# doubleailes/crust-render

Hardware: AMD Instinct MI355X
Metric: Mray/s (closest-hit + shadow queries) of the path-tracing integrator (higher is better)
Workload: dtype f32; 1 GPU; samples/cornellbox.usda 1920x1080, 512 spp per step per GPU-share (x1 GPUs), depth 32, triangle r=1, variance 0; 14 steps = 7168 spp; rays_total=33550217735, closest_hit=33550217735, camera_rays=14863564800, target_spp=1024

## Files before the change

crust-render_amd/__init__.py:

```python
import ctypes as C
import os
import subprocess

import numpy as np

_HERE = os.path.dirname(os.path.abspath(__file__))
LIB_PATH = os.environ.get("CRT_AMD_LIB") or os.path.join(_HERE, "libcrt_amd.so")
CSRC = os.path.join(_HERE, "csrc")

MASK_CAMERA, MASK_SHADOW, MASK_INDIRECT, MASK_ALL = 1, 2, 4, 0xFFFFFFFF
INVALID_ID = 0xFFFFFFFF
INF = float("inf")

CRT_OK = 0
_ERRORS = {-1: "CRT_ERR_BAD_ARG", -2: "CRT_ERR_BAD_ID", -3: "CRT_ERR_NO_DEVICE", -4: "CRT_ERR_STACK",
           -5: "CRT_ERR_UNSUPPORTED", -6: "CRT_ERR_NO_MEMORY"}


class CrtError(RuntimeError):
    def __init__(self, code, what=""):
        detail = ""
        try:
            detail = _lib.crt_last_error().decode() if _lib is not None else ""
        except Exception:
# ... 677 lines not shown
            lib().crt_environment_free(h)

    def __del__(self):
        try:
            self.free()
        except Exception:
            pass

    def tables(self):
        t = CrtEnvironmentTables()
        _check(lib().crt_environment_tables(self.h, C.byref(t)), "crt_environment_tables")
        w, h = int(t.width), int(t.height)
        arr = lambda p, *shape: np.ctypeslib.as_array(p, shape=shape).copy()
        return dict(width=w, height=h, id=int(t.id), marginal_integral=np.float32(t.marginal_integral),
                    marginal_func=arr(t.marginal_func, h), marginal_cdf=arr(t.marginal_cdf, h + 1),
                    conditional_func=arr(t.conditional_func, h, w), conditional_cdf=arr(t.conditional_cdf, h, w + 1),
                    conditional_integral=arr(t.conditional_integral, h),
                    light_to_world=np.array(t.light_to_world, dtype=np.float32).reshape(3, 3).T.copy(),
                    world_to_light=np.array(t.world_to_light, dtype=np.float32).reshape(3, 3).T.copy(),
                    image=np.ctypeslib.as_array(C.cast(t.image, C.POINTER(C.c_uint8)), shape=(int(t.image_bytes),)).copy())


def environment_of(d):
    env = d.get("environment")
    if env is None or isinstance(env, Environment):
        return env
    return Environment(env["width"], env["height"], env["rgb"], env.get("light_to_world"))


def make_lights(light_dicts):
    arr = (CrtLight * max(len(light_dicts), 1))()
    keep = []
    for k, d in enumerate(light_dicts):
        l = arr[k]
        if d["kind"] == "dome" and d.get("environment") is not None:
            env = environment_of(d)
            tint = np.asarray(d["radiance"], dtype=np.float32)
            _check(lib().crt_light_dome_mapped(C.byref(l), _fp(tint), env.h), "crt_light_dome_mapped")
            keep.append(env)
            continue
        l.kind = {"sphere": LIGHT_SPHERE, "rect": LIGHT_RECT, "distant": LIGHT_DISTANT,
                  "dome": LIGHT_DOME}[d["kind"]]
        l.geom_id = int(d["geom_id"])
        l.radiance[:] = [float(x) for x in d["radiance"]]
        if d["kind"] == "distant":
            l.normal[:] = [float(x) for x in d["direction"]]
            l.radius = float(d["cos_half_angle"])
            l.center[0] = float(d["solid_angle"])
        elif d["kind"] == "dome":
            pass
        elif d["kind"] == "sphere":
            l.center[:] = [float(x) for x in d["center"]]
            l.radius = float(d["radius"])
        else:
            for f in ("origin", "edge_u", "edge_v", "normal"):
                getattr(l, f)[:] = [float(x) for x in d[f]]
    arr._environments = keep
    return arr


class Renderer:

    def __init__(self, scene, materials, lights, camera, settings, rank=0, world=1):
        self.scene = scene
        n = len(materials)
        self._mats = (CrtMaterial * max(n, 1))(*materials)
        self._lights = lights if not isinstance(lights, (list, tuple)) else make_lights(lights)
        self.n_lights = len(lights)
        self.settings = settings
        cs = settings.c()
        self.h = lib().crt_renderer_new(scene.h, self._mats, n, self._lights, self.n_lights, C.byref(camera),
                                        C.byref(cs), rank, world)
        if not self.h:
            raise CrtError(-1, "crt_renderer_new")
        self.n_pix = lib().crt_renderer_pixel_count(self.h)
        self.volumes = None

    def __del__(self):
        try:
            if self.h:
                lib().crt_renderer_free(self.h)
        except Exception:
            pass

    def pixel_indices(self):
        out = np.zeros(self.n_pix, dtype=np.uint32)
        _check(lib().crt_renderer_pixel_indices(self.h, _up(out)), "crt_renderer_pixel_indices")
        return out

    def render_samples(self, sample_begin, sample_count, stream=None):
        _check(lib().crt_render_samples(self.h, sample_begin, sample_count, _stream_ptr(stream)), "crt_render_samples")

    def set_volumes(self, vol):
        _check(lib().crt_renderer_set_volumes(self.h, vol.h if vol is not None else None), "crt_renderer_set_volumes")
        self.volumes = vol

    def render_samples_stats(self, sample_begin, sample_count, stream=None):
        st = (CrtTravStats * 2)()
        _check(lib().crt_render_samples_stats(self.h, sample_begin, sample_count, _stream_ptr(stream), st),
               "crt_render_samples_stats")
        return st[0], st[1]

    def film_to(self, d_rgb, stream=None):
        _check(lib().crt_film_resolve(self.h, d_rgb.data_ptr(), _stream_ptr(stream)), "crt_film_resolve")

    def film(self):
        out = np.zeros((self.n_pix, 3), dtype=np.float32)
        _check(lib().crt_film_read(self.h, _fp(out)), "crt_film_read")
        return out

    def image(self):
        img = np.zeros((self.settings.height * self.settings.width, 3), dtype=np.float32)
        img[self.pixel_indices()] = self.film()
        return img.reshape(self.settings.height, self.settings.width, 3)

    def clear(self, stream=None):
        _check(lib().crt_film_clear(self.h, _stream_ptr(stream)), "crt_film_clear")

    def stats(self):
        s = CrtRayStats()
        _check(lib().crt_render_stats(self.h, C.byref(s)), "crt_render_stats")
        return s

    def active_pixels(self):
        return int(lib().crt_renderer_active_pixels(self.h))

    def sample_counts(self):
        out = np.zeros(self.n_pix, dtype=np.uint32)
        _check(lib().crt_renderer_sample_counts(self.h, out.ctypes.data_as(C.POINTER(C.c_uint32))), "crt_renderer_sample_counts")
        return out

    def render_adaptive(self, spp, first=None, batch=4, stream=None):
        first = first or -(-max(self.settings.min_spp, 2) // 4) * 4
        s = 0
        while s < spp and self.active_pixels() > 0:
            n = min(first if s == 0 else batch, spp - s)
            self.render_samples(s, n, stream)
            s += n
        return s

    SHADE_CLASSES = ("emissive / escaped", "base", "coat / fuzz / thin film", "transmissive / subsurface")

    def shade_class_stats(self, enable=None):
        w, l = (C.c_uint64 * 4)(), (C.c_uint64 * 4)()
        _check(lib().crt_renderer_shade_class_stats(self.h, -1 if enable is None else int(bool(enable)), w, l),
               "crt_renderer_shade_class_stats")
        return {n: (int(w[k]), (l[k] / (64.0 * w[k])) if w[k] else 0.0) for k, n in enumerate(self.SHADE_CLASSES)}

    def pipeline(self):
        out = (C.c_uint32 * 3)()
        _check(lib().crt_renderer_pipeline(self.h, out), "crt_renderer_pipeline")
        return dict(fused=bool(out[0]), wide=bool(out[1] & 1), shade_pipe=bool(out[1] & 2), root_cull=bool(out[1] & 4),
                    slim_state=bool(out[1] & 8), volumes=bool(out[1] & 16), camera_trace=bool(out[1] & 32),
                    camera_vertex=bool(out[1] & 64), grid=int(out[2]))

    def lanes(self):
        return int(lib().crt_renderer_lanes(self.h)) if hasattr(lib(), "crt_renderer_lanes") else 1

    def set_lanes(self, lanes):
        return _check(lib().crt_renderer_set_lanes(self.h, int(lanes)), "crt_renderer_set_lanes")

    def profile(self, enable=True):
        _check(lib().crt_renderer_profile(self.h, 1 if enable else 0), "crt_renderer_profile")

    def profile_read(self):
        ms = (C.c_double * 4)()
        n = (C.c_uint64 * 4)()
        _check(lib().crt_renderer_profile_read(self.h, ms, n), "crt_renderer_profile_read")
        names = ("extend", "shade", "shadow", "other")
        return {names[k]: dict(ms=float(ms[k]), launches=int(n[k])) for k in range(4)}


def scene_path(name):
    import os
    if str(name).startswith("synthetic:") or os.path.exists(name):
        return name
    base = os.path.join(os.path.dirname(os.path.dirname(os.path.abspath(__file__))), "scenes", name)
    for ext in (".usda", ".usd", ".usda.xz"):
        if os.path.exists(base + ext):
            return base + ext
    raise FileNotFoundError("no scene %r under scenes/" % name)


def load_usda(path, width=None, height=None, max_depth=None, rank=0, world=1, variance=0.0, min_spp=None, dist=None,
              timings=None, cubic_curves=False, environment_maps=False):
    from . import usda, shard
    import sys
    import time
    t0 = time.perf_counter()
    if str(path).startswith("synthetic:"):
        from . import synthetic
        parts = str(path).split(":")
        kw = dict(side=int(parts[2])) if len(parts) > 2 else {}
        desc = getattr(synthetic, parts[1])(width or 640, height or 360, **kw)
    else:
        desc = shard.import_once(path, width, height, dist, cubic_curves=cubic_curves, environment_maps=environment_maps)
    me = sys.modules[__name__]
    t1 = time.perf_counter()
    scene, materials, protos = usda.build_world(desc, me, default_material)
    t2 = time.perf_counter()
    if timings is not None:
        timings.update(import_s=t1 - t0, commit_s=t2 - t1)
    s = desc.settings
    settings = RenderSettings(s["width"], s["height"], s["max_depth"] if max_depth is None else max_depth, s["frame"],
                              s["strategy"], s["filter"], s["filter_radius"], float(variance),
                              s["min_spp"] if min_spp is None else min_spp)
    cam = make_camera(**desc.camera)
    r = Renderer(scene, materials, desc.lights, cam, settings, rank, world)
    r._protos = protos
    return r, desc

def render_with_report(path, spp=None, out_exr=None, width=None, height=None, max_depth=None, variance=None,
                       batch=16, volumes=False):
    import sys
    from . import stats as _stats
    st = _stats.RenderStats()
    me = sys.modules[__name__]
    with st.phase("Parse USD stage"):
        desc = usda.load(path, width, height, volumes=bool(volumes))
    s = desc.settings
    with st.phase("Commit acceleration structure"):
        scene, materials, protos = usda.build_world(desc, me, default_material)
        scene.memory_footprint()
    var = s["variance"] if variance is None else variance
    settings = RenderSettings(s["width"], s["height"], s["max_depth"] if max_depth is None else max_depth, s["frame"],
                              s["strategy"], s["filter"], s["filter_radius"], float(var), s["min_spp"])
    r = Renderer(scene, materials, desc.lights, make_camera(**desc.camera), settings)
    r._protos = protos
    vol = usda.build_volumes(desc, me) if volumes else None
    if vol is not None:
        r.set_volumes(vol)
    n = int(spp if spp is not None else s["spp"])
    with st.phase("Render"):
        if var > 0:
            r.render_adaptive(n, batch=batch)
        else:
            for b in range(0, n, 32):
                r.render_samples(b, min(32, n - b))
        img = r.image()
    if out_exr:
        with st.phase("Write image"):
            exr.write_exr(out_exr, img[::-1])
    _stats.for_render(scene, r, n, st)
    return img, st


load_scene = load_usda

from . import usda
from . import usdc
from . import shard
from . import exr
from . import stats
from . import shading
from . import volumes
from . import guiding
from . import synthetic
```

crust-render_amd/csrc/crt_internal.h:

```cpp
#pragma once

#include <atomic>
#include <cmath>
#include <cstddef>
#include <cstdint>
#include <memory>
#include <mutex>
#include <vector>

#include "../../include/crt.h"
#include "../../include/crt_render_volumes.h"
#include "../../include/crt_scene_image.h"

namespace crt {

struct F3 {
  float x, y, z;
  float operator[](int i) const { return i == 0 ? x : (i == 1 ? y : z); }
  float &at(int i) { return i == 0 ? x : (i == 1 ? y : z); }
};
inline F3 f3(float x, float y, float z) { return F3{x, y, z}; }
inline F3 operator+(F3 a, F3 b) { return {a.x + b.x, a.y + b.y, a.z + b.z}; }
inline F3 operator-(F3 a, F3 b) { return {a.x - b.x, a.y - b.y, a.z - b.z}; }
inline F3 operator*(F3 a, float s) { return {a.x * s, a.y * s, a.z * s}; }
// ... 182 lines not shown
inline bool wide_split(const DevScene &s, bool renderer = false) {
  if (s.direct_leaves != 0 || s.n_packets == 0) return false;
  if (s.pool_stack >= 10u) return renderer && s.n_nodes > 2048u;
  return s.n_nodes <= 1024u;
}

#ifndef CRT_POOL_STACK
#define CRT_POOL_STACK 6
#endif
#ifndef CRT_POOL_STACK_DEEP
#define CRT_POOL_STACK_DEEP 10
#endif
#ifndef CRT_POOL_STACK_WIDE
#define CRT_POOL_STACK_WIDE 3
#endif

struct EngineSelect {
  bool wide = false;
  bool wide_direct = false;
  bool direct = false;
  uint32_t lds_stack = CRT_POOL_STACK;
  uint32_t window = CRT_POOL_NODES;
  int ext_cold = (int)kColdAll;
  int path_cold = (int)kColdAll;
  bool curve = false;
  bool cubic = false;
  int curve_cold() const { return (int)((curve ? kColdCurve : 0u) | (cubic ? kColdCubic : 0u)); }
};
inline int select_engine(const DevScene &s, int want_wide, EngineSelect &e, bool renderer = false) {
  const bool has_direct_words = s.direct_leaves != 0;
  const bool curve = (s.cold & kColdCurve) != 0;
  if (curve && want_wide > 0) return CRT_ERR_UNSUPPORTED;
  if (want_wide == 1 && has_direct_words) return CRT_ERR_UNSUPPORTED;
  if (want_wide == 2 && !(has_direct_words && renderer && CRT_DIRECT_LEAVES != 0 && CRT_WIDE_DIRECT_BUILD != 0)) return CRT_ERR_UNSUPPORTED;
  const bool auto_wide_direct = !curve && want_wide < 0 && renderer && has_direct_words && CRT_DIRECT_LEAVES != 0 && CRT_WIDE_DIRECT_BUILD != 0;
  e.wide = auto_wide_direct || (want_wide < 0 ? (!curve && wide_split(s, renderer)) : want_wide != 0);
  e.wide_direct = auto_wide_direct || want_wide == 2;
  e.direct = (!e.wide || e.wide_direct) && CRT_DIRECT_LEAVES != 0 && has_direct_words;
  if (has_direct_words && !e.direct) return CRT_ERR_UNSUPPORTED;
  const bool deep = s.pool_stack >= (uint32_t)CRT_POOL_STACK_DEEP;
  e.lds_stack = e.wide ? (uint32_t)CRT_POOL_STACK_WIDE + 1u + (deep ? 1u : 0u) : (deep ? (uint32_t)CRT_POOL_STACK_DEEP : (uint32_t)CRT_POOL_STACK);
  e.window = e.wide ? (deep ? (uint32_t)CRT_POOL_NODES_WIDE_DEEP : (uint32_t)CRT_POOL_NODES_WIDE)
                    : (deep ? (uint32_t)CRT_POOL_NODES_DEEP : (uint32_t)CRT_POOL_NODES);
  const int cold = (int)(s.cold & kColdAll);
  e.ext_cold = cold == 0 ? 0 : (cold == (int)kColdNormal ? (int)kColdNormal : (int)kColdAll);
  e.path_cold = cold == 0 ? 0 : (int)kColdAll;
  if (CRT_NOPK_BUILD && s.n_packets == 0 && e.direct) e.path_cold = (int)(kColdAll | kNoPackets);
  e.curve = curve;
  e.cubic = curve && (s.cold & kColdCubic) != 0;
  if (curve) e.ext_cold = e.path_cold = (int)kColdAll | e.curve_cold();
  return CRT_OK;
}
inline bool engine_accepts(const EngineSelect &e, const DevScene &s, int kernel_cold) {
  if (s.direct_leaves != 0 && ((e.wide && !e.wide_direct) || !e.direct)) return false;
  if (e.wide_direct && s.direct_leaves == 0) return false;
  if ((kernel_cold & (int)kNoPackets) && (s.n_packets != 0 || s.direct_leaves == 0)) return false;
  if ((s.cold & kColdCurve) && (e.wide || !e.curve)) return false;
  if ((s.cold & kColdCubic) && (e.wide || !e.cubic || !(s.cold & kColdCurve))) return false;
  return ((int)(s.cold & (kColdAll | kColdCurve | kColdCubic)) & ~kernel_cold) == 0;
}

enum KernelFamily : uint8_t { KF_NONE = 0, KF_EXTEND, KF_PATH, KF_SHADE, KF_SHADE_ENV, KF_SHADE_PIPE, KF_SHADOW, KF_SHADOW_CURVE, KF_SHADOW_CUBIC,
                               KF_SHADE_VOL, KF_VOLUME, KF_SHADOW_VOLUME, KF_EXTEND_DEFERRED };
struct InstanceKey {
  uint8_t family = KF_NONE;
  uint8_t arg[5] = {0, 0, 0, 0, 0};
  bool none() const { return family == KF_NONE; }
  bool operator==(const InstanceKey &o) const {
    return family == o.family && arg[0] == o.arg[0] && arg[1] == o.arg[1] && arg[2] == o.arg[2] && arg[3] == o.arg[3] && arg[4] == o.arg[4];
  }
};
#define CRT_INSTANCE_KEY(family, kernel, ...) ::crt::InstanceKey{::crt::KF_##family, {__VA_ARGS__}}
#if CRT_WIDE_DIRECT_BUILD
#define CRT_WIDE_DIRECT_INSTANCES_EXTEND(X) X(EXTEND, k_extend, false, 2, 0) X(EXTEND, k_extend, false, 2, 2) X(EXTEND, k_extend, false, 2, 7)
#define CRT_WIDE_DIRECT_INSTANCES_SHADOW(X) X(SHADOW, k_shadow, false, 2)
#else
#define CRT_WIDE_DIRECT_INSTANCES_EXTEND(X)
#define CRT_WIDE_DIRECT_INSTANCES_SHADOW(X)
#endif
#if CRT_NOPK_BUILD
#define CRT_NOPK_INSTANCES_PATH(X) X(PATH, k_path, 1, false, 15, false) X(PATH, k_path, 1, true, 15, false) X(PATH, k_path, 2, false, 15, false) X(PATH, k_path, 2, true, 15, false)
#else
#define CRT_NOPK_INSTANCES_PATH(X)
#endif
#define CRT_INSTANCES_EXTEND(X)  \
  X(EXTEND, k_extend, false, 0, 0) X(EXTEND, k_extend, false, 0, 2) X(EXTEND, k_extend, false, 0, 7) \
  X(EXTEND, k_extend, false, 1, 0) X(EXTEND, k_extend, false, 1, 2) X(EXTEND, k_extend, false, 1, 7) \
  CRT_WIDE_DIRECT_INSTANCES_EXTEND(X) \
  X(EXTEND, k_extend, true, 0, 7) X(EXTEND, k_extend, true, 1, 7) \
  X(EXTEND, k_extend, false, 0, 23) X(EXTEND, k_extend, true, 0, 23) X(EXTEND, k_extend, false, 0, 55) X(EXTEND, k_extend, true, 0, 55)
#define CRT_INSTANCES_EXTEND_DEFERRED(X)  \
  X(EXTEND_DEFERRED, k_extend_deferred, false, 1, 0)
#define CRT_INSTANCES_PATH(X)  \
  X(PATH, k_path, 0, false, 0, true) X(PATH, k_path, 0, false, 7, true) X(PATH, k_path, 0, true, 0, true) X(PATH, k_path, 0, true, 7, true) \
  X(PATH, k_path, 0, false, 0, false) X(PATH, k_path, 0, false, 7, false) X(PATH, k_path, 0, true, 0, false) X(PATH, k_path, 0, true, 7, false) \
  X(PATH, k_path, 1, false, 7, false) X(PATH, k_path, 1, false, 23, false) X(PATH, k_path, 1, false, 55, false) \
  X(PATH, k_path, 1, true, 7, false) X(PATH, k_path, 1, true, 23, false) X(PATH, k_path, 1, true, 55, false) \
  X(PATH, k_path, 2, false, 7, false) X(PATH, k_path, 2, false, 23, false) X(PATH, k_path, 2, false, 55, false) \
  X(PATH, k_path, 2, true, 7, false) X(PATH, k_path, 2, true, 23, false) X(PATH, k_path, 2, true, 55, false) \
  CRT_NOPK_INSTANCES_PATH(X)
#define CRT_INSTANCES_SHADE(X)  \
  X(SHADE, k_shade, 0, false, false, false, true) X(SHADE, k_shade, 0, false, false, true, true) X(SHADE, k_shade, 0, false, true, false, true) \
  X(SHADE, k_shade, 0, false, true, true, true) X(SHADE, k_shade, 0, true, false, true, true) \
  X(SHADE, k_shade, 0, false, false, false, false) X(SHADE, k_shade, 0, false, false, true, false) X(SHADE, k_shade, 0, false, true, false, false) \
  X(SHADE, k_shade, 0, false, true, true, false) X(SHADE, k_shade, 0, true, false, true, false) \
  X(SHADE, k_shade, 1, false, false, false, false) X(SHADE, k_shade, 1, false, false, true, false) X(SHADE, k_shade, 1, true, false, true, false) \
  X(SHADE, k_shade, 2, false, false, false, false) X(SHADE, k_shade, 2, false, false, true, false) X(SHADE, k_shade, 2, true, false, true, false) \
  X(SHADE_ENV, k_shade_env, 0, true) X(SHADE_ENV, k_shade_env, 0, false) X(SHADE_ENV, k_shade_env, 1, false) X(SHADE_ENV, k_shade_env, 2, false)
#define CRT_INSTANCES_SHADE_PIPE(X)  \
  X(SHADE_PIPE, k_shade_pipe, true) X(SHADE_PIPE, k_shade_pipe, false)
#define CRT_INSTANCES_SHADE_PIPE_SLIM(X)  \
  X(SHADE_PIPE, k_shade_pipe, true, true) X(SHADE_PIPE, k_shade_pipe, false, true)
#define CRT_INSTANCES_SHADOW(X)  \
  X(SHADOW, k_shadow, false, 0) X(SHADOW, k_shadow, false, 1) CRT_WIDE_DIRECT_INSTANCES_SHADOW(X) X(SHADOW, k_shadow, true, 0) X(SHADOW, k_shadow, true, 1) \
  X(SHADOW_CURVE, k_shadow_curve, false) X(SHADOW_CURVE, k_shadow_curve, true) X(SHADOW_CUBIC, k_shadow_cubic, false) X(SHADOW_CUBIC, k_shadow_cubic, true)
#define CRT_INSTANCES_SHADE_VOL(X)  \
  X(SHADE_VOL, k_shade_vol, 0, 0, false) X(SHADE_VOL, k_shade_vol, 0, 0, true) X(SHADE_VOL, k_shade_vol, 0, 1, true) X(SHADE_VOL, k_shade_vol, 0, 2, true) \
  X(SHADE_VOL, k_shade_vol, 1, 0, false) X(SHADE_VOL, k_shade_vol, 1, 0, true) X(SHADE_VOL, k_shade_vol, 1, 1, true) X(SHADE_VOL, k_shade_vol, 1, 2, true) \
  X(SHADE_VOL, k_shade_vol, 2, 0, false) X(SHADE_VOL, k_shade_vol, 2, 0, true) X(SHADE_VOL, k_shade_vol, 2, 1, true) X(SHADE_VOL, k_shade_vol, 2, 2, true)

struct PlanInputs {
  EngineSelect engine;
  DevScene scene{};
  int mats_kind = 1;
  bool mat_derived = true;
  uint32_t n_lights = 0;
  bool has_inf_lights = false, has_env = false;
  uint32_t strategy = 0;
  bool has_motion = false, lens = false;
  bool mat_index = false;
  uint32_t partition = 0, class_stats = 0, n_materials = 0, max_depth = 0;
  int force_fused = -1;
  bool prefer_stage = true;
  size_t stage_min_paths = (size_t)96 << 20;
  int tail_from = 12;
  int noclassify_from = 1 << 30;
  int shade_wide = -1;
  int shade_pipe = 1;
  int slim_state = 1;
  bool no_emitter = false;
  bool cam_compact_ok = true;
  int root_cull_knob = -1;
  float root_miss_share = 0.0f;
  bool volumes = false;
  int camera_trace_knob = -1;
  size_t total = 0;
  bool stats = false;
  bool partial_active = false;
  bool cam_compact_build = true, wide_direct_build = CRT_WIDE_DIRECT_BUILD != 0, nopk_build = CRT_NOPK_BUILD != 0;
  bool shade_pipe_build = true, root_cull_build = true;
  int pipe_mat_max = 0;
  bool camera_trace_build = true;
  int camera_vertex_knob = -1;
};
constexpr uint32_t kCameraTraceMaxNodes = 1024;
constexpr float kRootCullMinShare = 0.125f;
inline bool shade_pipe_fits(const PlanInputs &q) {
  return q.shade_pipe_build && q.shade_pipe != 0 && q.mats_kind == 0 && q.n_lights == 0 && !q.has_motion && !q.mat_index &&
         q.partition == 0 && !q.class_stats && q.n_materials <= (uint32_t)q.pipe_mat_max;
}
inline bool table_has_no_emitter(const CrtMaterial *m, size_t n) {
  auto finite = [](float x) { return x - x == 0.0f; };
  for (size_t k = 0; k < n; k++) {
    const float *c = m[k].emission_color, lum = m[k].emission_luminance;
    const bool emissive = m[k].kind == CRT_MAT_EMISSIVE;
    const bool black = c[0] == 0.0f && c[1] == 0.0f && c[2] == 0.0f && (emissive ? lum == lum : finite(lum));
    const bool dark = !emissive && lum == 0.0f && finite(c[0]) && finite(c[1]) && finite(c[2]);
    if (!black && !dark) return false;
  }
  return true;
}
struct LaunchPlan {
  bool fused = true;
  bool wide = false;
  uint32_t tail_at = 0xffffffffu;
  uint32_t cam_compact = 0;
  bool root_cull = false;
  bool shadow = false;
  int noclassify_from = 1 << 30;
  int ext_cold = 0, path_cold = 0;
  InstanceKey path, extend, shade, shade_early, shadow_key;
  bool shade_piped() const { return !shade_early.none(); }
  bool volumes = false;
  InstanceKey volume_key, shadow_volume_key;
  bool camera_trace = false;
  uint32_t camera_mode = 0;
  InstanceKey extend_deferred_key() const {
    InstanceKey k = camera_trace ? extend : InstanceKey{};
    if (camera_trace) k.family = KF_EXTEND_DEFERRED;
    return k;
  }
  bool slim_state = false;
  InstanceKey shade_slim_key() const {
    InstanceKey k = slim_state ? shade_early : InstanceKey{};
    if (slim_state) k.arg[1] = 1;
    return k;
  }
  bool camera_vertex = false;
};
inline EngineSelect engine_of_width(const EngineSelect &e, const DevScene &s, int w) {
  EngineSelect l = e;
  l.wide = w != 0;
  l.wide_direct = w == 2;
  l.direct = w != 1 && CRT_DIRECT_LEAVES != 0 && s.direct_leaves != 0;
  return l;
}
inline int plan_launches(const PlanInputs &q, LaunchPlan &out) {
  const EngineSelect &e = q.engine;
  LaunchPlan pl;
  pl.fused = q.force_fused >= 0 ? q.force_fused != 0 : !(q.prefer_stage && q.total >= q.stage_min_paths);
  if (q.stats || q.has_inf_lights) pl.fused = false;
  if (q.volumes) pl.fused = false;
  pl.volumes = q.volumes;
  const bool stage = !pl.fused, lit = q.n_lights > 0;
  pl.wide = stage && e.wide;
  const bool tail = stage && q.tail_from > 0 && !q.stats && !q.has_inf_lights && !q.volumes;
  if (tail) pl.tail_at = (uint32_t)q.tail_from;
  pl.cam_compact = (q.cam_compact_build && stage && q.cam_compact_ok && !lit && !q.lens && !q.has_motion && !q.volumes) ? 1u : 0u;
  pl.root_cull = q.root_cull_build && q.root_cull_knob != 0 && (q.root_cull_knob > 0 || q.root_miss_share >= kRootCullMinShare) &&
                 stage && !q.stats && q.scene.root != CRT_INVALID_ID && q.max_depth > 0 && !q.has_inf_lights &&
                 !q.volumes;
  if (pl.root_cull && pl.cam_compact) pl.cam_compact = q.mats_kind == 0 ? 2u : 0u;
  pl.shadow = stage && lit && q.strategy != CRT_STRATEGY_BSDF;
  pl.noclassify_from = q.noclassify_from;
  const int curve_cold = e.curve ? (int)kColdAll | e.curve_cold() : 0;
  const bool simple = q.mats_kind == 0, drv = simple && q.mat_derived;
  pl.ext_cold = e.curve ? curve_cold : (q.stats ? (int)kColdAll : e.ext_cold);
  pl.path_cold = e.curve ? curve_cold : (simple ? (e.path_cold & (int)kColdAll) : (int)kColdAll | (q.nopk_build ? e.path_cold & (int)kNoPackets : 0));
  auto key = [](KernelFamily f, int a0, int a1 = 0, int a2 = 0, int a3 = 0, int a4 = 0) {
    InstanceKey k;
    k.family = f;
    k.arg[0] = (uint8_t)a0; k.arg[1] = (uint8_t)a1; k.arg[2] = (uint8_t)a2; k.arg[3] = (uint8_t)a3; k.arg[4] = (uint8_t)a4;
    return k;
  };
  const bool wdirect = pl.wide && e.wide_direct && q.wide_direct_build;
  const int width = e.curve ? 0 : (wdirect ? (q.stats ? 0 : 2) : (pl.wide ? 1 : 0));
  int shadow_cold = (int)kColdAll;
  if (pl.fused || tail)
    pl.path = key(KF_PATH, q.mats_kind, lit, simple && pl.path_cold != 0 ? (int)kColdAll : pl.path_cold, drv);
  if (stage) {
    pl.extend = key(KF_EXTEND, q.stats, width, pl.ext_cold);
    const bool shade_wide = simple && !q.has_inf_lights && pl.wide && !q.mat_index && q.shade_wide != 0;
    pl.shade = q.has_env ? key(KF_SHADE_ENV, q.mats_kind, drv) : key(KF_SHADE, q.mats_kind, q.has_inf_lights, shade_wide, lit, drv);
    if (q.volumes) {
      pl.shade = key(KF_SHADE_VOL, q.mats_kind, q.has_env ? 2 : (q.has_inf_lights ? 1 : 0), lit);
      pl.volume_key = key(KF_VOLUME, 0);
      if (pl.shadow) pl.shadow_volume_key = key(KF_SHADOW_VOLUME, 0);
    } else if (shade_wide && shade_pipe_fits(q) && q.noclassify_from > 0) pl.shade_early = key(KF_SHADE_PIPE, drv);
    pl.slim_state = pl.shade_piped() && q.no_emitter && q.slim_state != 0;
    if (pl.shadow) {
      if (e.curve) { pl.shadow_key = key(e.cubic ? KF_SHADOW_CUBIC : KF_SHADOW_CURVE, q.stats); shadow_cold = curve_cold; }
      else pl.shadow_key = key(KF_SHADOW, q.stats, width);
    }
    pl.camera_trace = q.camera_trace_build && q.camera_trace_knob != 0 && !q.stats && !q.volumes && !q.partial_active &&
                      pl.cam_compact != 0 && width == 1 && pl.ext_cold == 0 && q.max_depth >= 1 && q.scene.root != CRT_INVALID_ID &&
                      q.scene.n_packets > 0 && q.scene.has_packets != 0 && q.scene.direct_leaves == 0 &&
                      (q.camera_trace_knob > 0 || q.scene.n_nodes <= kCameraTraceMaxNodes);
    if (pl.camera_trace) pl.camera_mode = q.camera_trace_knob == 2 ? 1u : (q.camera_trace_knob == 3 ? (1u << 8) : 0u);
    pl.camera_vertex = pl.camera_trace && pl.shade_piped() && q.max_depth >= 1 && q.camera_vertex_knob != 0;
  }
  const bool ok = !(q.volumes && q.stats) &&
                  (pl.path.none() || engine_accepts(engine_of_width(e, q.scene, 0), q.scene, pl.path.arg[2])) &&
                  (pl.extend.none() || engine_accepts(engine_of_width(e, q.scene, width), q.scene, pl.extend.arg[2])) &&
                  (pl.shadow_key.none() || engine_accepts(engine_of_width(e, q.scene, width), q.scene, shadow_cold));
  if (!ok) { pl.path = pl.extend = pl.shade = pl.shade_early = pl.shadow_key = pl.volume_key = pl.shadow_volume_key = InstanceKey{}; pl.slim_state = false; pl.camera_trace = false; pl.camera_mode = 0; pl.camera_vertex = false; }
  out = pl;
  return ok ? CRT_OK : CRT_ERR_UNSUPPORTED;
}

int wide_request();

struct Knobs {
  int pool_stack_deep = -1;
  int direct_leaves = -1;
  int direct_inst = -1;
  int stage_roots = -1;
  uint32_t cold = 0;
  int inst_order = 1;
  int hot_packets = 1;
  int wide = -1;
  int mat_dedup = 1, partition = -1, simple = 1, prefer_stage = -1, cam_compact = 1, root_cull = -1, shade_wide = -1, shade_pipe = 1, fused = -1;
  int mat_derived = 1;
  int slim_state = 1;
  int camera_trace = -1;
  int camera_vertex = -1;
  int noclassify_from = 1 << 30, tail_from = 12, lanes = 4, grid_mult = 0;
  size_t max_batch_slots = 0, lane_min_paths = (size_t)96 << 20, stage_min_paths = (size_t)96 << 20;
};
Knobs read_knobs();
inline int select_engine_env(const DevScene &s, EngineSelect &e, bool renderer = false) {
  if (select_engine(s, wide_request(), e, renderer) == CRT_OK) return CRT_OK;
  return select_engine(s, -1, e, renderer);
}

struct DeviceImage {
  void *blob = nullptr;
  size_t bytes[7] = {0, 0, 0, 0, 0, 0, 0};
  uint32_t *err = nullptr;
  DevScene view{};
  ~DeviceImage();
};

struct Scene : std::enable_shared_from_this<Scene> {
  Bvh bvh;
  uint32_t n_geoms = 0;
  bool has_motion = false;
  uint32_t depth = 1;
  std::mutex dev_mu;
  std::unique_ptr<DeviceImage> dev;
  int ensure_device();
};

int scene_image_check(const Scene &scene, uint64_t out[8]);
int scene_image_prims(const Scene &scene, std::vector<DevPrim> &out);
int scene_image_array(const Scene &scene, uint32_t which, std::vector<unsigned char> &out, uint32_t view[8]);
int scene_root_touched(const Scene &scene, const float *rays6, size_t n, float t_min, float t_max, uint8_t *out, uint32_t *root);
int scene_engine_select(const Scene &scene, int want_wide, uint32_t out[8]);

enum GeomKind { G_MESH, G_SPHERE, G_INSTANCE, G_CURVES, G_CUBICS };
struct Geom {
  GeomKind kind = G_MESH;
  uint32_t mask = CRT_MASK_ALL;
  std::vector<float> verts;
  std::vector<uint32_t> idx;
  bool has_normals = false;
  std::vector<float> normals;
  F3 center{0, 0, 0};
  float radius = 0;
  std::vector<float> segs;
  std::shared_ptr<Scene> scene;
  Affine l2w{};
  bool has_end = false;
  Affine l2w_end{};
};

struct Builder { std::vector<Geom> geoms; };

std::shared_ptr<Scene> commit(Builder &&b);

int launch_intersect_n(const DevScene &s, const CrtRay *d_rays, size_t n, float t_min, float t_max, CrtRayHit *d_hits,
                       void *stream, CrtTravStats *d_stats, uint32_t *d_err);
int launch_occluded_n(const DevScene &s, const CrtRay *d_rays, size_t n, float t_min, float t_max, uint32_t *d_out,
                      void *stream, CrtTravStats *d_stats, uint32_t *d_err);
int device_ok();
int env_table_for_launch(const void **table);
std::shared_ptr<void> env_retain(uint32_t id);
namespace dev { struct VolRegionRec; }
struct VolumesView { const dev::VolRegionRec *regions = nullptr; const float *grid = nullptr; uint32_t n_regions = 0; };
int volumes_build_image(const CrtVolumeRegion *regions, size_t n, const float *grid, size_t grid_len, std::vector<unsigned char> &image);
int volumes_device(CrtVolumes *v, VolumesView &out);
void volumes_retain(CrtVolumes *v);
void volumes_release(CrtVolumes *v);
uint32_t volumes_region_count(const CrtVolumes *v);
void set_error_text(const char *fmt, ...);
template <class F>
inline int abi_guard(const char *what, F &&body) noexcept {
  try { return body(); }
  catch (const std::exception &e) { set_error_text("%s: %s", what, e.what()); }
  catch (...) { set_error_text("%s: unknown failure", what); }
  return CRT_ERR_NO_MEMORY;
}

bool hip_failed(int  err, const char *what, const char *file, int line);
#define CRT_HIP_OK(call) (!::crt::hip_failed((int)(call), #call, __FILE__, __LINE__))

}

struct CrtScene { std::shared_ptr<crt::Scene> p; std::atomic<int> refs{1}; };
struct CrtBuilder { crt::Builder b; };
```

crust-render_amd/csrc/kernels/pathtrace.hip:

```cpp
#include <cstddef>
#include <cstdlib>
#include <cstring>
#include <new>
#include <string>
#include <unordered_map>
#include <vector>

#include "shade.hip.h"
#include "traverse_camera.hip.h"
#include "traverse_pool.hip.h"
#include "vertex_simple.hip.h"
#include "volume.hip.h"

namespace crt {

using namespace dev;

namespace {

#ifndef CRT_EXTEND_WAVES
#define CRT_EXTEND_WAVES 3
#endif
#ifndef CRT_SHADE_WAVES
#define CRT_SHADE_WAVES 3
#endif
#ifndef CRT_SHADOW_WAVES
#define CRT_SHADOW_WAVES 3
#endif

enum { K_CAMERA = 0, K_PATH = 1, K_TIME = 2 };
constexpr uint32_t kFilmTarget = 0x80000000u;
constexpr uint32_t kPrevValid = 1u << 16, kPrevDelta = 1u << 17;
constexpr int kMediumShift = 18;
constexpr uint32_t kMaxMedia = (1u << 14) - 1;
constexpr uint32_t kVolScatter = 0xfffffff0u;
__device__ __forceinline__ bool vol_scatter_word(uint32_t hg) { return hg >= kVolScatter && hg < kVolScatter + 4u; }

#ifndef CRT_NT
#define CRT_NT 1
#endif
typedef float nt_f4 __attribute__((ext_vector_type(4)));
typedef uint32_t nt_u4 __attribute__((ext_vector_type(4)));
__device__ __forceinline__ void st_nt(float4 *p, float4 v) {
  if (CRT_NT) { nt_f4 x = {v.x, v.y, v.z, v.w}; __builtin_nontemporal_store(x, reinterpret_cast<nt_f4 *>(p)); }
  else *p = v;
}
__device__ __forceinline__ void st_nt(uint4 *p, uint4 v) {
  if (CRT_NT) { nt_u4 x = {v.x, v.y, v.z, v.w}; __builtin_nontemporal_store(x, reinterpret_cast<nt_u4 *>(p)); }
  else *p = v;
}
__device__ __forceinline__ void st_nt(uint32_t *p, uint32_t v) {
  if (CRT_NT) __builtin_nontemporal_store(v, p);
  else *p = v;
}
__device__ __forceinline__ void st_nt(float *p, float v) {
  if (CRT_NT) __builtin_nontemporal_store(v, p);
  else *p = v;
}
#ifndef CRT_NT_HIT
#define CRT_NT_HIT CRT_NT
#endif
__device__ __forceinline__ void st_hit(float4 *p, float4 v) { if (CRT_NT_HIT) st_nt(p, v); else *p = v; }
__device__ __forceinline__ void st_hit(uint32_t *p, uint32_t v) { if (CRT_NT_HIT) st_nt(p, v); else *p = v; }
__device__ __forceinline__ float4 ld_nt(const float4 *p) {
  if (CRT_NT) { const nt_f4 x = __builtin_nontemporal_load(reinterpret_cast<const nt_f4 *>(p)); return make_float4(x.x, x.y, x.z, x.w); }
  return *p;
}

struct PathSoA {
  float4 *a;
  float4 *b;
  float4 *c;
  uint4 *d;
  float4 *e;
  float *time;
};
struct HitSoA { float4 *h; uint32_t *geom; };
struct ShadowSoA { float4 *a, *b, *c; };

#ifndef CRT_BINS
#define CRT_BINS 1
#endif
constexpr int kBins = CRT_BINS;
constexpr int kMaxGrid = 16384;
struct Counters {
  uint32_t err;
  uint32_t pad;
  unsigned long long stats[8];
  uint32_t seg[2][kMaxGrid * kBins];
  uint32_t shadow[kMaxGrid];
  unsigned long long cls_waves[4], cls_lanes[4];
  uint32_t cam_defer[kMaxGrid];
};

__device__ __forceinline__ uint32_t dir_bin(float dx, float dy, float dz) {
  if (kBins == 1) return 0;
  return (dx < 0.0f ? 1u : 0u) | (dy < 0.0f ? 2u : 0u) | (dz < 0.0f ? 4u : 0u);
}
__device__ __forceinline__ void bins_prefix(const uint32_t *counts, uint32_t *pre ) {
  if (threadIdx.x == 0) {
    uint32_t acc = 0;
    for (int b = 0; b < kBins; b++) { pre[b] = acc; acc += ((const volatile uint32_t *)counts)[b]; }
    pre[kBins] = acc;
  }
  __syncthreads();
}
__device__ __forceinline__ uint32_t bin_slot(uint32_t k, const uint32_t *pre, uint32_t seg_cap) {
  uint32_t b = 0;
#pragma unroll
  for (int t = 1; t < kBins; t++) b += k >= pre[t] ? 1u : 0u;
  return (blockIdx.x * kBins + b) * seg_cap + (k - pre[b]);
}

struct Params {
  DevScene scene;
  uint32_t sample_begin;
  const CrtMaterial *materials;
  const DevMaterial *mat_derived;
  uint32_t n_materials;
  const uint16_t *mat_index;
  const DevMedium *media;
  const DevMedium *media_by_id;
  const CrtLight *lights;
  uint32_t n_lights;
  uint32_t has_inf_lights;
  CrtCamera camera;
  uint32_t width, height, max_depth;
  int32_t frame, strategy, filter_kind;
  float filter_radius;
  uint32_t has_motion;
  const uint32_t *pixel_index;
  uint32_t n_pix;
  const uint32_t *active;
  uint32_t n_act;
  uint32_t seg_cap;
  const uint8_t *mat_class;
  uint32_t partition;
  uint32_t class_stats;
  uint32_t cam_compact;
  uint32_t root_cull;
  const EnvSlot *envs;
};

__device__ __forceinline__ float light_weight(int s, float light_pdf, float bounce_pdf) {
  switch (s) {
    case CRT_STRATEGY_POWER: return power_heuristic(light_pdf, bounce_pdf);
    case CRT_STRATEGY_BALANCE: return balance_heuristic(light_pdf, bounce_pdf);
    case CRT_STRATEGY_LIGHT: return 1.0f;
    default: return 0.0f;
  }
}
__device__ __forceinline__ float bounce_weight(int s, float bounce_pdf, float light_pdf) {
  switch (s) {
    case CRT_STRATEGY_POWER: return power_heuristic(bounce_pdf, light_pdf);
    case CRT_STRATEGY_BALANCE: return balance_heuristic(bounce_pdf, light_pdf);
    case CRT_STRATEGY_LIGHT: return 0.0f;
    default: return 1.0f;
  }
}
__device__ __forceinline__ V3 sky_gradient(V3 unit_direction) {
  const float t = 0.5f * (unit_direction.y + 1.0f);
  return v3(1.0f, 1.0f, 1.0f) * (1.0f - t) + v3(0.5f, 0.7f, 1.0f) * t;
}
__device__ __forceinline__ V3 escaped_to_sky(V3 rd, V3 beta, V3 L) {
  const V3 unit_direction = normalize(rd);
  const V3 background = splat(0.0f) + sky_gradient(unit_direction);
  return L + beta * background;
}
template <bool ENV = false>
__device__ __forceinline__ V3 escaped_background(const CrtLight *lights, uint32_t n_lights, int strategy,
                                                 V3 unit_direction, bool competing, float prev_pdf, const EnvSlot *envs = nullptr) {
  V3 background = splat(0.0f);
  bool covered = false;
  for (uint32_t k = 0; k < n_lights; k++) {
    V3 emitted;
    float pdf;
    if (!light_escaped_env<ENV>(lights[k], envs, unit_direction, emitted, pdf)) continue;
    covered = true;
    float weight = 1.0f;
    if (competing && strategy != CRT_STRATEGY_BSDF) {
      const float light_pdf = rmax(pdf / (float)n_lights, 1e-6f);
      weight = bounce_weight(strategy, prev_pdf, light_pdf);
    }
    background = background + emitted * weight;
  }
  if (!covered) background = background + sky_gradient(unit_direction);
  return background;
}

__device__ __forceinline__ bool lds_take(bool want, uint32_t *next, uint32_t limit, uint32_t &idx) {
  const unsigned long long mask = __ballot(want);
  if (mask == 0) return false;
  const int lane = threadIdx.x & 63;
  const int leader = __ffsll((long long)mask) - 1;
  uint32_t base = 0;
  if (lane == leader) base = atomicAdd(next, (uint32_t)__popcll(mask));
  base = __shfl(base, leader, 64);
  idx = base + (uint32_t)__popcll(mask & ((1ull << lane) - 1ull));
  return want && idx < limit;
}

__device__ __forceinline__ uint32_t seg_append(bool want, uint32_t *lds_counter) {
  const unsigned long long mask = __ballot(want);
  if (mask == 0) return 0;
  const int lane = threadIdx.x & 63;
  const int leader = __ffsll((long long)mask) - 1;
  uint32_t base = 0;
  if (lane == leader) base = atomicAdd(lds_counter, (uint32_t)__popcll(mask));
  base = __shfl(base, leader, 64);
  return base + (uint32_t)__popcll(mask & ((1ull << lane) - 1ull));
}

__device__ __forceinline__ void add_stat(uint32_t *lds_slot, uint32_t v) {
  for (int off = 32; off > 0; off >>= 1) v += __shfl_down(v, off, 64);
  if ((threadIdx.x & 63) == 0 && v) atomicAdd(lds_slot, v);
}

__global__ void k_build_media(const CrtMaterial *materials, uint32_t n, DevMedium *media) {
  const uint32_t i = blockIdx.x * blockDim.x + threadIdx.x;
  if (i >= n) return;
  DevMedium m;
  medium_from_material(materials[i], m);
  m.id = 0;
  media[i] = m;
}
__global__ void k_derive_materials(const CrtMaterial *materials, uint32_t n, DevMaterial *derived) {
  const uint32_t i = blockIdx.x * blockDim.x + threadIdx.x;
  if (i >= n) return;
  DevMaterial d;
  derive_material(materials[i], d);
  derived[i] = d;
}
template <bool DRV> struct MatTable;
template <> struct MatTable<false> {
  typedef CrtMaterial Rec;
  __device__ __forceinline__ static const Rec *of(const Params &P) { return P.materials; }
  __device__ __forceinline__ static MatRaw view(const Rec *table, const Params &, uint32_t i) { return MatRaw{table[i]}; }
};
template <> struct MatTable<true> {
  typedef DevMaterial Rec;
  __device__ __forceinline__ static const Rec *of(const Params &P) { return P.mat_derived; }
  __device__ __forceinline__ static MatDerived view(const Rec *table, const Params &P, uint32_t i) { return MatDerived{table[i], P.materials[i]}; }
};
constexpr int kNumberBlock = 1024;
__global__ __launch_bounds__(kNumberBlock) void k_number_media(uint32_t n, DevMedium *media, DevMedium *by_id, uint32_t *count_out) {
  __shared__ uint32_t run_sum[kNumberBlock];
  const uint32_t per = (n + kNumberBlock - 1) / kNumberBlock;
  const uint32_t lo = threadIdx.x * per < n ? threadIdx.x * per : n, hi = lo + per < n ? lo + per : n;
  uint32_t mine = 0;
  for (uint32_t i = lo; i < hi; i++) mine += media[i].present ? 1u : 0u;
  run_sum[threadIdx.x] = mine;
  __syncthreads();
  for (int off = 1; off < kNumberBlock; off <<= 1) {
    const uint32_t add = (int)threadIdx.x >= off ? run_sum[threadIdx.x - off] : 0u;
    __syncthreads();
    run_sum[threadIdx.x] += add;
    __syncthreads();
  }
  uint32_t count = run_sum[threadIdx.x] - mine;
  for (uint32_t i = lo; i < hi; i++) {
    if (!media[i].present) continue;
    count++;
    if (count <= kMaxMedia) {
      media[i].id = count;
      by_id[count - 1] = media[i];
    }
  }
  if (threadIdx.x == kNumberBlock - 1) *count_out = run_sum[threadIdx.x];
}

constexpr int kArenaDwords = kEngineLdsDwords > kSobolLdsWords ? kEngineLdsDwords : kSobolLdsWords;
static_assert(sizeof(CrtMaterial) % 4 == 0, "material records are copied as dwords");
constexpr int kClasses = 4;
constexpr uint32_t kRing = 2 * kBlock;
constexpr int kRingDwords = kClasses * (int)kRing;
constexpr int kClassLdsMax = 1024;
constexpr int mat_lds_max(int arena) { return (arena - kSobolLdsWords - kRingDwords - kClassLdsMax / 4) / (int)(sizeof(CrtMaterial) / 4); }
#ifndef CRT_SHADE_WIDE_WAVES
#define CRT_SHADE_WIDE_WAVES 4
#endif
constexpr int kArenaWide = (160 / CRT_SHADE_WIDE_WAVES) * 1024 / 4 - 256;
static_assert(mat_lds_max(kArenaWide) >= 16 && mat_lds_max(kArenaDwords) >= 16, "the arena holds the Sobol tables, the rings and a material table");

inline uint8_t material_class(const CrtMaterial &m) {
  if (m.kind == CRT_MAT_EMISSIVE) return 0;
  if (m.transmission_weight > 0.0f || m.subsurface_weight > 0.0f) return 3;
  if (m.coat_weight > 0.0f || m.fuzz_weight > 0.0f || m.thin_film_weight > 0.0f) return 2;
  return 1;
}

struct CameraSample { V3 o, d; float time; uint32_t pattern, pix, sl; };
__device__ __forceinline__ CameraSample camera_sample(const Params &P, size_t g, uint32_t sample_begin, const uint32_t *sobol_tab) {
  CameraSample cs;
  cs.pix = (uint32_t)(g % P.n_act); cs.sl = (uint32_t)(g / P.n_act);
  const uint32_t lin = P.pixel_index[P.active ? P.active[cs.pix] : cs.pix];
  const uint32_t px = lin % P.width, py = lin / P.width;
  const int tile = (int)(px >> 8) + (int)(py >> 8) * 4096;
  const Sampler root = new_domain(sampler_new((int)px, (int)py, P.frame, (int)(sample_begin + cs.sl)), tile);
  float cam[4];
  draw_sample4(new_domain(root, K_CAMERA), cam, sobol_tab);
  const float fx = filter_offset(P.filter_kind, P.filter_radius, cam[0]);
  const float fy = filter_offset(P.filter_kind, P.filter_radius, cam[1]);
  const float u = ((float)px + fx) / (float)P.width;
  const float v = ((float)py + fy) / (float)P.height;
  cs.time = 0.0f;
  if (P.has_motion) {
    float t4[4];
    draw_sample4(new_domain(root, K_TIME), t4, sobol_tab);
    cs.time = t4[0];
  }
  camera_get_ray(P.camera, u, v, cam[2], cam[3], cs.o, cs.d);
  cs.pattern = new_domain(root, K_PATH).pattern;
  return cs;
}
__device__ __forceinline__ size_t camera_slot_sample(size_t k) {
  return ((k / kBlock) * (size_t)gridDim.x + blockIdx.x) * kBlock + (k % kBlock);
}

template <bool PLANE_D>
__device__ __forceinline__ void compact_camera_path(const Params &P, uint32_t k, float4 a, float4 &A, float4 &B, uint4 &D) {
  const V3 o = ld3(P.camera.origin) + splat(0.0f);
  A = make_float4(o.x, o.y, o.z, a.x);
  B = make_float4(a.y, a.z, 1.0f, 1.0f);
  if (PLANE_D && P.cam_compact == 2) return;
  const uint32_t g = (uint32_t)camera_slot_sample(k);
  D = make_uint4(__float_as_uint(a.w), g % P.n_act, (P.max_depth & 0xffffu) << 16, g / P.n_act);
}

#ifndef CRT_REGEN_FIRST
#define CRT_REGEN_FIRST 0
#endif
constexpr bool kRegenFirst = CRT_REGEN_FIRST != 0;
#ifndef CRT_CAM_COMPACT_BUILD
#define CRT_CAM_COMPACT_BUILD 1
#endif
#ifndef CRT_MAT_INDEX_BUILD
#define CRT_MAT_INDEX_BUILD 1
#endif
static_assert(kBins == 1 || !CRT_REGEN_FIRST, "the first shade takes a camera path's sample number from its slot: one sub-segment per workgroup");
__device__ __forceinline__ void generate_segment(const Params &P, const PathSoA &S, Counters *C, uint32_t sample_begin,
                                                 uint32_t n_samples, uint32_t *sobol_tab , bool write_c) {
  sobol_tables_init(sobol_tab);
  const size_t total = (size_t)P.n_act * n_samples;
  const size_t seg0 = (size_t)blockIdx.x * kBins * P.seg_cap;
  uint32_t seg_n = 0;
  for (size_t k = threadIdx.x; k < P.seg_cap; k += kBlock) {
    const size_t g = camera_slot_sample(k);
    if (g >= total) break;
    seg_n = (uint32_t)k + 1;
    const size_t i = seg0 + k;
    const CameraSample cs = camera_sample(P, g, sample_begin, sobol_tab);
    if (CRT_CAM_COMPACT_BUILD && !write_c && P.cam_compact) {
      st_nt(&S.a[i], make_float4(cs.d.x, cs.d.y, cs.d.z, __uint_as_float(cs.pattern)));
      continue;
    }
    st_nt(&S.a[i], make_float4(cs.o.x, cs.o.y, cs.o.z, cs.d.x));
    st_nt(&S.b[i], make_float4(cs.d.y, cs.d.z, 1.0f, 1.0f));
    if (write_c) st_nt(&S.c[i], make_float4(1.0f, 0.0f, 0.0f, 0.0f));
    if (write_c || !kRegenFirst) st_nt(&S.d[i], make_uint4(cs.pattern, cs.pix, (P.max_depth & 0xffffu) << 16, cs.sl));
    if (P.has_motion) st_nt(&S.time[i], cs.time);
  }
  __shared__ uint32_t seg_max;
  if (threadIdx.x == 0) seg_max = 0;
  __syncthreads();
  if (seg_n) atomicMax(&seg_max, seg_n);
  __syncthreads();
  if (threadIdx.x == 0) {
    for (int b = 0; b < kBins; b++) {
      C->seg[0][blockIdx.x * kBins + b] = b == 0 ? seg_max : 0;
      C->seg[1][blockIdx.x * kBins + b] = 0;
    }
    C->shadow[blockIdx.x] = 0;
    if (blockIdx.x == 0) atomicAdd(&C->stats[0], (unsigned long long)total);
  }
}
constexpr bool kRootCullBuild = kBins == 1 && !kRegenFirst;
__device__ __forceinline__ void generate_segment_cull(const Params &P, const PathSoA &S, Counters *C, uint32_t sample_begin,
                                                      uint32_t n_samples, uint32_t *sobol_tab , float4 *staging) {
  float bmin[3][4], bmax[3][4];
  uint32_t child[4];
  {
    const WideNode &root = P.scene.nodes[P.scene.root];
#pragma unroll
    for (int a = 0; a < 3; a++)
#pragma unroll
      for (int l = 0; l < 4; l++) { bmin[a][l] = root.bmin[a][l]; bmax[a][l] = root.bmax[a][l]; }
#pragma unroll
    for (int l = 0; l < 4; l++) child[l] = root.child[l];
  }
  __shared__ uint32_t cull_ctr[2];
  if (threadIdx.x < 2) cull_ctr[threadIdx.x] = 0;
  sobol_tables_init(sobol_tab);
  const size_t total = (size_t)P.n_act * n_samples;
  const size_t seg0 = (size_t)blockIdx.x * kBins * P.seg_cap;
  const bool compact = CRT_CAM_COMPACT_BUILD && P.cam_compact != 0;
  uint32_t n_culled = 0;
  for (size_t k0 = 0; k0 < P.seg_cap; k0 += kBlock) {
    if (camera_slot_sample(k0) >= total) break;
    const size_t g = camera_slot_sample(k0 + threadIdx.x);
    CameraSample cs;
    cs.o = splat(0.0f); cs.d = splat(0.0f); cs.time = 0.0f; cs.pattern = 0; cs.pix = 0; cs.sl = 0;
    bool keep = false;
    if (g < total) {
      cs = camera_sample(P, g, sample_begin, sobol_tab);
      keep = node_touched(bmin, bmax, child, cs.o.x, cs.o.y, cs.o.z, cs.d.x, cs.d.y, cs.d.z, 0.001f, CRT_INF);
      if (!keep) {
        const V3 L = escaped_to_sky(cs.d, splat(1.0f), splat(0.0f));
        st_nt(&staging[cs.sl * P.n_act + cs.pix], make_float4(L.x, L.y, L.z, 0.0f));
        n_culled++;
      }
    }
    const size_t i = seg0 + seg_append(keep, &cull_ctr[0]);
    if (keep) {
      const uint4 D = make_uint4(cs.pattern, cs.pix, (P.max_depth & 0xffffu) << 16, cs.sl);
      if (compact) {
        st_nt(&S.a[i], make_float4(cs.d.x, cs.d.y, cs.d.z, __uint_as_float(cs.pattern)));
        st_nt(&S.d[i], D);
      } else {
        st_nt(&S.a[i], make_float4(cs.o.x, cs.o.y, cs.o.z, cs.d.x));
        st_nt(&S.b[i], make_float4(cs.d.y, cs.d.z, 1.0f, 1.0f));
        st_nt(&S.d[i], D);
        if (P.has_motion) st_nt(&S.time[i], cs.time);
      }
    }
  }
  add_stat(&cull_ctr[1], n_culled);
  __syncthreads();
  if (threadIdx.x == 0) {
    for (int b = 0; b < kBins; b++) {
      C->seg[0][blockIdx.x * kBins + b] = b == 0 ? cull_ctr[0] : 0;
      C->seg[1][blockIdx.x * kBins + b] = 0;
    }
    C->shadow[blockIdx.x] = 0;
    if (blockIdx.x == 0) atomicAdd(&C->stats[0], (unsigned long long)total);
    if (cull_ctr[1]) {
      atomicAdd(&C->stats[1], (unsigned long long)cull_ctr[1]);
      atomicAdd(&C->stats[6], (unsigned long long)cull_ctr[1]);
    }
  }
}
__global__ __launch_bounds__(kBlock) void k_generate(Params P, PathSoA S, Counters *C, uint32_t sample_begin,
                                                     uint32_t n_samples, float4 *staging) {
  __shared__ uint32_t sobol_tab[kSobolLdsWords];
  if (kRootCullBuild && P.root_cull) generate_segment_cull(P, S, C, sample_begin, n_samples, sobol_tab, staging);
  else generate_segment(P, S, C, sample_begin, n_samples, sobol_tab, false);
}

constexpr int kCamLdsDwords = kCamWindow * kLdsNodeStride + kCamStack * kBlock;
static_assert((kSobolLdsWords + kCamLdsDwords) * 4 + 512 <= 40 * 1024, "four workgroups of k_camera per CU");
__global__ __launch_bounds__(kBlock, 4) void k_camera(Params P, PathSoA S, uint32_t *defer_plane, HitSoA H, Counters *C,
                                                      uint32_t sample_begin, uint32_t n_samples, float4 *staging, uint32_t mode) {
  __shared__ uint32_t sobol_tab[kSobolLdsWords];
  __shared__ __attribute__((aligned(16))) uint32_t cam_lds[kCamLdsDwords];
  __shared__ uint32_t cam_ctr[3];
  const bool cull = P.root_cull != 0;
  float bmin[3][4], bmax[3][4];
  uint32_t child[4];
  {
    const WideNode &root = P.scene.nodes[P.scene.root];
#pragma unroll
    for (int a = 0; a < 3; a++)
#pragma unroll
      for (int l = 0; l < 4; l++) { bmin[a][l] = root.bmin[a][l]; bmax[a][l] = root.bmax[a][l]; }
#pragma unroll
    for (int l = 0; l < 4; l++) child[l] = root.child[l];
  }
  if (threadIdx.x < 3) cam_ctr[threadIdx.x] = 0;
  uint32_t *lds_nodes = cam_lds;
  uint32_t *stk = cam_lds + kCamWindow * kLdsNodeStride + threadIdx.x;
  uint32_t n_lds_pk;
  const uint32_t n_lds = stage_nodes(P.scene, lds_nodes, kCamWindow, n_lds_pk);
  sobol_tables_init(sobol_tab);
  const bool defer_all = (mode & 1u) != 0;
  const uint32_t want_stack = mode >> 8;
  const uint32_t pstack = (want_stack == 0 || want_stack > (uint32_t)kCamStack) ? (uint32_t)kCamStack : want_stack;
  const size_t total = (size_t)P.n_act * n_samples;
  const size_t seg0 = (size_t)blockIdx.x * kBins * P.seg_cap;
  uint32_t *list = defer_plane + 4 * seg0;
  const V3 cam_o = ld3(P.camera.origin) + splat(0.0f);
  uint32_t n_culled = 0, n_valid = 0;
  for (size_t k0 = 0; k0 < P.seg_cap; k0 += kBlock) {
    if (camera_slot_sample(k0) >= total) break;
    const size_t g = camera_slot_sample(k0 + threadIdx.x);
    CameraSample cs;
    cs.o = splat(0.0f); cs.d = splat(0.0f); cs.time = 0.0f; cs.pattern = 0; cs.pix = 0; cs.sl = 0;
    bool keep = false;
    if (g < total) {
      cs = camera_sample(P, g, sample_begin, sobol_tab);
      keep = true;
      n_valid = (uint32_t)(k0 + threadIdx.x) + 1;
      if (cull) {
        keep = node_touched(bmin, bmax, child, cs.o.x, cs.o.y, cs.o.z, cs.d.x, cs.d.y, cs.d.z, 0.001f, CRT_INF);
        if (!keep) {
          const V3 L = escaped_to_sky(cs.d, splat(1.0f), splat(0.0f));
          st_nt(&staging[cs.sl * P.n_act + cs.pix], make_float4(L.x, L.y, L.z, 0.0f));
          n_culled++;
        }
      }
    }
    uint32_t at = (uint32_t)(k0 + threadIdx.x);
    if (cull) at = seg_append(keep, &cam_ctr[0]);
    const size_t i = seg0 + at;
    int res = CAM_MISS;
    if (keep) {
      st_nt(&S.a[i], make_float4(cs.d.x, cs.d.y, cs.d.z, __uint_as_float(cs.pattern)));
      if (P.cam_compact == 2) st_nt(&S.d[i], make_uint4(cs.pattern, cs.pix, (P.max_depth & 0xffffu) << 16, cs.sl));
      float t = 0.0f;
      uint32_t prim = kInvalid;
      res = defer_all ? (int)CAM_DEFER
                      : camera_trace(P.scene, lds_nodes, n_lds, n_lds_pk, stk, kBlock, pstack, 0.001f, CRT_INF, CRT_MASK_CAMERA,
                                     cam_o.x, cam_o.y, cam_o.z, cs.d.x, cs.d.y, cs.d.z, t, prim);
      if (res == CAM_HIT) {
        float4 h;
        uint32_t gw;
        camera_hit_record(P.scene, prim, t, cs.d.x, cs.d.y, cs.d.z, h, gw);
        st_hit(&H.h[i], h);
        st_hit(&H.geom[i], gw);
      } else if (res == CAM_MISS) {
        st_hit(&H.geom[i], kInvalid);
      }
    }
    const bool later = keep && res == CAM_DEFER;
    const uint32_t li = seg_append(later, &cam_ctr[2]);
    if (later) list[li] = (uint32_t)i;
  }
  add_stat(&cam_ctr[1], n_culled);
  if (!cull && n_valid) atomicMax(&cam_ctr[0], n_valid);
  __syncthreads();
  if (threadIdx.x == 0) {
    for (int b = 0; b < kBins; b++) {
      C->seg[0][blockIdx.x * kBins + b] = b == 0 ? cam_ctr[0] : 0;
      C->seg[1][blockIdx.x * kBins + b] = 0;
    }
    C->shadow[blockIdx.x] = 0;
    C->cam_defer[blockIdx.x] = cam_ctr[2];
    if (blockIdx.x == 0) atomicAdd(&C->stats[0], (unsigned long long)total);
    if (cam_ctr[1]) {
      atomicAdd(&C->stats[1], (unsigned long long)cam_ctr[1]);
      atomicAdd(&C->stats[6], (unsigned long long)cam_ctr[1]);
    }
  }
}

template <bool STATS, int WIDE, int COLD, bool COMPACT, bool DEFER = false>
__device__ __forceinline__ void extend_segment(const Params &P, const PathSoA &S, const HitSoA &H, Counters *C, int cur,
                                               int first, CrtTravStats *tstats, uint32_t *engine_lds,
                                               const uint32_t *defer_list = nullptr) {
  __shared__ uint32_t pre[kBins + 1];
  bins_prefix(&C->seg[cur][blockIdx.x * kBins], pre);
  const uint32_t n = DEFER ? C->cam_defer[blockIdx.x] : pre[kBins];
  if (n == 0) return;
  __shared__ uint32_t next;
  if (threadIdx.x == 0) next = 0;
  LaneStats st = {};
  uint32_t err = 0, done = 0;
  const uint32_t mask = first ? CRT_MASK_CAMERA : CRT_MASK_INDIRECT;
  auto fetch = [&](bool want, RayIn &in) -> bool {
    uint32_t k;
    if (!lds_take(want, &next, n, k)) return false;
    const uint32_t i = DEFER ? defer_list[4 * (size_t)blockIdx.x * kBins * P.seg_cap + k] : bin_slot(k, pre, P.seg_cap);
    if (CRT_CAM_COMPACT_BUILD && COMPACT && first && P.cam_compact) {
      const float4 A = ld_nt(&S.a[i]);
      const V3 o = ld3(P.camera.origin) + splat(0.0f);
      in.ox = o.x; in.oy = o.y; in.oz = o.z; in.dx = A.x; in.dy = A.y; in.dz = A.z;
      in.time = 0.0f;
    } else {
      const float4 A = ld_nt(&S.a[i]), B = ld_nt(&S.b[i]);
      in.ox = A.x; in.oy = A.y; in.oz = A.z; in.dx = A.w; in.dy = B.x; in.dz = B.y;
      in.time = P.has_motion ? S.time[i] : 0.0f;
    }
    in.mask = mask; in.t_min = 0.001f; in.t_max = CRT_INF; in.slot = i;
    return true;
  };
  auto emit = [&](uint32_t i, bool hit, const Hit &h, float dx, float dy, float dz) {
    if (hit) {
      const bool front = dot3(dx, dy, dz, h.nx, h.ny, h.nz) < 0.0f;
      st_hit(&H.h[i], make_float4(h.t, front ? h.nx : -h.nx, front ? h.ny : -h.ny, front ? h.nz : -h.nz));
      st_hit(&H.geom[i], h.geom | (front ? 0x80000000u : 0u));
    } else {
      st_hit(&H.geom[i], kInvalid);
    }
    done++;
  };
  run_traversal<false, STATS, WIDE, COLD, WIDE != 0>(P.scene, engine_lds, 0.001f, err, st, fetch, emit, mask);
  if (err) atomicOr(&C->err, err);
  if (STATS) flush_stats(st, tstats, done);
}
template <bool STATS, int WIDE, int COLD>
__global__ __launch_bounds__(kBlock, WIDE ? 4 : CRT_EXTEND_WAVES) void k_extend(Params P, PathSoA S, HitSoA H, Counters *C, int cur,
                                                                     int first, CrtTravStats *tstats) {
  __shared__ __attribute__((aligned(16))) uint32_t engine_lds[WIDE ? kEngineLdsWide : kEngineLdsDwords];
  extend_segment<STATS, WIDE, COLD, true>(P, S, H, C, cur, first, tstats, engine_lds);
}
template <bool STATS, int WIDE, int COLD>
__global__ __launch_bounds__(kBlock, WIDE ? 4 : CRT_EXTEND_WAVES) void k_extend_deferred(Params P, PathSoA S, HitSoA H, Counters *C, int cur,
                                                                              int first, CrtTravStats *tstats, const uint32_t *defer_list) {
  __shared__ __attribute__((aligned(16))) uint32_t engine_lds[WIDE ? kEngineLdsWide : kEngineLdsDwords];
  extend_segment<STATS, WIDE, COLD, true, true>(P, S, H, C, cur, first, tstats, engine_lds, defer_list);
}

#ifndef CRT_SHADE_STAMPS
#define CRT_SHADE_STAMPS 0
#endif
template <int MATS, int INF, bool LIT, int ARENA, bool DRV, bool VOL = false>
__device__ __forceinline__ void shade_segment(const Params &P, const PathSoA &S, const PathSoA &N, const HitSoA &H,
                                              const ShadowSoA &Q, Counters *C, int cur, float4 *staging,
                                              uint32_t *sobol_tab ,
                                              bool first ,
                                              bool all_pending = false ,
                                              uint32_t *qseed = nullptr ) {
  constexpr bool MEDIA = MATS == 2, SIMPLE = MATS == 0;
  static_assert(SIMPLE || !DRV, "the derived record covers what a simple-material table reads (shade.hip.h)");
  typedef MatTable<DRV> Table;
  constexpr bool COMPACT = CRT_CAM_COMPACT_BUILD && !LIT;
  constexpr bool COMPACT_D = COMPACT && SIMPLE;
  constexpr bool MAT_INDEX = CRT_MAT_INDEX_BUILD && ARENA != kArenaWide;
  __shared__ uint32_t lds_ctr[10];
  __shared__ uint32_t out_n[kBins];
  __shared__ uint32_t pre[kBins + 1];
  bins_prefix(&C->seg[cur][blockIdx.x * kBins], pre);
  const uint32_t n = pre[kBins];
  if (n == 0) {
    if (threadIdx.x < kBins) C->seg[1 - cur][blockIdx.x * kBins + threadIdx.x] = 0;
    if (threadIdx.x == 0) C->shadow[blockIdx.x] = 0;
    return;
  }
  if (threadIdx.x < 10) lds_ctr[threadIdx.x] = 0;
  if (threadIdx.x < kBins) out_n[threadIdx.x] = 0;
  sobol_tables_init(sobol_tab);
  const typename Table::Rec *mats = Table::of(P);
  if (P.n_materials <= (uint32_t)mat_lds_max(ARENA)) {
    uint32_t *dst = sobol_tab + kSobolLdsWords;
    const uint32_t *src = reinterpret_cast<const uint32_t *>(mats);
    const uint32_t words = P.n_materials * (uint32_t)(sizeof(CrtMaterial) / 4);
    for (uint32_t w = threadIdx.x; w < words; w += kBlock) dst[w] = src[w];
    mats = reinterpret_cast<const typename Table::Rec *>(dst);
    __syncthreads();
  }
  const uint32_t seg0 = blockIdx.x * P.seg_cap;
  const uint32_t n_lights = LIT ? P.n_lights : 0u;
  uint32_t s_closest = 0, s_shadow = 0, s_vertices = 0, s_rr_t = 0, s_rr_k = 0, s_esc = 0, s_depth = 0;
  uint32_t *ring = sobol_tab + ARENA - kRingDwords;
  uint8_t *cls_lds = reinterpret_cast<uint8_t *>(ring) - kClassLdsMax;
  __shared__ uint32_t ring_tail[kClasses];
  const bool part = P.partition != 0;
// ... 660 lines not shown
        hg = stg[1280 + lane];
      }
      asm volatile("s_waitcnt lgkmcnt(0)" ::: "memory");
    }
    lap(0);
    while (next_in < n && tail_h - head_h < (uint32_t)kBlock && tail_m - head_m < (uint32_t)kBlock) {
      lds_barrier();
      const uint32_t k_c = next_in + threadIdx.x;
      const uint32_t hg_c = hg_next;
      next_in += kBlock;
      hg_next = kInvalid;
      if (next_in + threadIdx.x < n) hg_next = H.geom[seg0 + next_in + threadIdx.x];
      const bool hit = k_c < n && hg_c != kInvalid, miss = k_c < n && hg_c == kInvalid;
      const uint32_t at_h = seg_append(hit, &ring_tail[0]);
      if (SLIM) { if (hit) reinterpret_cast<uint2 *>(ring_h)[at_h % kPipeRing] = make_uint2(k_c, hg_c); }
      else if (hit) ring_h[at_h % kPipeRing] = k_c;
      const uint32_t at_m = seg_append(miss, &ring_tail[1]);
      if (miss) ring_m[at_m % kPipeRing] = k_c;
      lds_barrier();
      tail_h = uniform(ring_tail[0]);
      tail_m = uniform(ring_tail[1]);
      if (STAMPS) t_acc[6]++;
    }
    lap(1);
    const uint32_t pend_h = tail_h - head_h, pend_m = tail_m - head_m;
    uint32_t kind_n = 0, take_n = 0, k_n = 0;
    if (pend_h >= (uint32_t)kBlock || (pend_h && pend_m < (uint32_t)kBlock)) { kind_n = 1; take_n = pend_h < (uint32_t)kBlock ? pend_h : (uint32_t)kBlock; }
    else if (pend_m) { kind_n = 2; take_n = pend_m < (uint32_t)kBlock ? pend_m : (uint32_t)kBlock; }
    const uint32_t head_n = head_h;
    if (SLIM && kind_n && threadIdx.x < take_n) {
      k_n = kind_n == 1 ? ring_h[2 * ((head_h + threadIdx.x) % kPipeRing)] : ring_m[(head_m + threadIdx.x) % kPipeRing];
      const uint32_t i_n = seg0 + k_n;
      lds_dma16(&S.a[i_n], stg);
      if (!first) {
        lds_dma16(&S.b[i_n], stg + 256);
        lds_dma16(&S.c[i_n], stg + 512);
      } else if (!compact) {
        lds_dma16(&S.b[i_n], stg + 256);
        lds_dma16(&S.d[i_n], stg + 512);
      } else if (compact_d) {
        lds_dma16(&S.d[i_n], stg + 512);
      }
      if (kind_n == 1 && !CRT_SHADE_PIPE_HIT_REGS) lds_dma16(&H.h[i_n], stg + 768);
    } else if (kind_n && threadIdx.x < take_n) {
      k_n = kind_n == 1 ? ring_h[(head_h + threadIdx.x) % kPipeRing] : ring_m[(head_m + threadIdx.x) % kPipeRing];
      const uint32_t i_n = seg0 + k_n;
      lds_dma16(&S.a[i_n], stg);
      if (!compact) {
        lds_dma16(&S.b[i_n], stg + 256);
        lds_dma16(&S.d[i_n], stg + 768);
        if (!first) lds_dma16(&S.c[i_n], stg + 512);
      } else if (compact_d) {
        lds_dma16(&S.d[i_n], stg + 768);
      }
      if (kind_n == 1 && !CRT_SHADE_PIPE_HIT_REGS) {
        lds_dma16(&H.h[i_n], stg + 1024);
        lds_dma4(&H.geom[i_n], stg + 1280);
      }
    }
    head_h += kind_n == 1 ? take_n : 0u;
    head_m += kind_n == 2 ? take_n : 0u;
    lap(2);
    const bool active = threadIdx.x < take;
    if (kind == 2) {
      if (active) {
        if (compact) compact_camera_path<true>(P, k_in, A, A, B, D);
        const int remaining = (int)(D.z >> 16);
        const V3 rd = v3(A.w, B.x, B.y), beta = v3(B.z, B.w, Cc.x);
        V3 L = v3(Cc.y, Cc.z, Cc.w);
        if (remaining > 0) {
          s_closest++;
          s_esc++;
          L = escaped_to_sky(rd, beta, L);
        } else {
          s_depth++;
          if ((D.w & kPrevValid) != 0) s_closest++;
        }
        st_nt(&staging[(D.w & 0xffffu) * P.n_act + D.y], make_float4(L.x, L.y, L.z, 0.0f));
      }
      lap(4);
    } else if (kind == 1) {
      bool alive = false;
      V3 L = splat(0.0f), beta = splat(1.0f), n_o = splat(0.0f), n_d = splat(0.0f);
      uint32_t meta = 0, aux = 0, pix = 0, pattern = 0;
      bool n_delta = false;
      if (active) {
        if (compact) compact_camera_path<true>(P, k_in, A, A, B, D);
        const V3 ro = v3(A.x, A.y, A.z), rd = v3(A.w, B.x, B.y);
        beta = v3(B.z, B.w, Cc.x);
        L = v3(Cc.y, Cc.z, Cc.w);
        pattern = D.x; pix = D.y; meta = D.z; aux = D.w;
        const uint32_t n_rec = meta & 0xffffu;
        const int remaining = (int)(meta >> 16);
        const bool prev_valid = (aux & kPrevValid) != 0;
        const uint32_t mat_i = hg & 0x7fffffffu;
        HitRec rec;
        rec.front_face = ((hg >> 31) & 1u) != 0;
        rec.t = hh.x;
        rec.normal = v3(hh.y, hh.z, hh.w);
        rec.p = ro + rd * rec.t;
        const auto mat = MatTable<DRV>::view(mats, P, mat_i);
        const VertexOut v = vertex_simple(mat, ro, rd, beta, L, rec, pattern, P.sample_begin + (aux & 0xffffu), n_rec, remaining,
                                          prev_valid, arena);
        beta = v.beta; L = v.L;
        alive = v.alive;
        n_o = v.origin; n_d = v.dir; n_delta = v.delta;
        s_closest += v.closest; s_vertices += v.vertices; s_rr_t += v.rr_tested; s_rr_k += v.rr_killed; s_esc += v.escaped;
        s_depth += v.depth_ended;
      }
      const uint32_t j = seg0 + seg_append(alive, &out_n);
      const uint32_t sl = aux & 0xffffu;
      if (alive) {
        st_nt(&N.a[j], make_float4(n_o.x, n_o.y, n_o.z, n_d.x));
        st_nt(&N.b[j], make_float4(n_d.y, n_d.z, beta.x, beta.y));
        if (SLIM && !out_full) {
          st_nt(&N.c[j], make_float4(beta.z, __uint_as_float(pattern), __uint_as_float(pix | (n_delta ? 0x80000000u : 0u)), __uint_as_float(sl)));
        } else {
          st_nt(&N.c[j], make_float4(beta.z, L.x, L.y, L.z));
          st_nt(&N.d[j], make_uint4(pattern, pix, ((meta & 0xffffu) + 1u) | (((meta >> 16) - 1u) << 16),
                                    sl | kPrevValid | (n_delta ? kPrevDelta : 0u)));
        }
      } else if (active) {
        st_nt(&staging[sl * P.n_act + pix], make_float4(L.x, L.y, L.z, 0.0f));
      }
      lap(3);
    }
    if (STAMPS) t_acc[5]++;
    if (!kind_n) break;
    kind = kind_n; take = take_n; k_in = k_n; head_in = head_n;
  }
  add_stat(&lds_ctr[2], s_closest); add_stat(&lds_ctr[4], s_vertices);
  add_stat(&lds_ctr[5], s_rr_t); add_stat(&lds_ctr[6], s_rr_k); add_stat(&lds_ctr[7], s_esc);
  add_stat(&lds_ctr[8], s_depth);
  __syncthreads();
  if (threadIdx.x == 0) {
    C->shadow[blockIdx.x] = 0;
    C->seg[1 - cur][blockIdx.x] = out_n;
    C->seg[cur][blockIdx.x] = 0;
  }
  if (threadIdx.x >= 1 && threadIdx.x <= 7 && lds_ctr[threadIdx.x + 1])
    atomicAdd(&C->stats[threadIdx.x], (unsigned long long)lds_ctr[threadIdx.x + 1]);
  if (STAMPS && lane == 0)
    for (int s = 0; s < 7; s++) atomicAdd(s < 4 ? &C->cls_waves[s] : &C->cls_lanes[s - 4], t_acc[s]);
}
template <bool DRV, bool SLIM = false>
__global__ __launch_bounds__(kBlock, CRT_SHADE_WIDE_WAVES) void k_shade_pipe(Params P, PathSoA S, PathSoA N, HitSoA H, Counters *C,
                                                                              int cur, float4 *staging, int first, uint32_t it,
                                                                              int out_full) {
  __shared__ __attribute__((aligned(16))) uint32_t arena[kArenaWide];
  shade_segment_pipe<DRV, SLIM>(P, S, N, H, C, cur, staging, arena, (first & 1) != 0, it, out_full != 0, (first & 2) != 0);
}

static_assert((kSobolLdsWords + kCamLdsDwords + kPipeMatMax * kMatDwords) * 4 + 512 <= 40 * 1024, "four workgroups of k_camera_vertex per CU");
template <bool DRV>
__global__ __launch_bounds__(kBlock, 4) void k_camera_vertex(Params P, PathSoA S, PathSoA N, Counters *C, uint32_t sample_begin,
                                                             uint32_t n_samples, float4 *staging, uint32_t mode, int slim_out) {
  __shared__ uint32_t sobol_tab[kSobolLdsWords];
  __shared__ __attribute__((aligned(16))) uint32_t cam_lds[kCamLdsDwords];
  __shared__ __attribute__((aligned(16))) uint32_t mat_lds[kPipeMatMax * kMatDwords];
  __shared__ uint32_t cam_ctr[4];
  const bool cull = P.root_cull != 0;
  float bmin[3][4], bmax[3][4];
  uint32_t child[4];
  {
    const WideNode &root = P.scene.nodes[P.scene.root];
#pragma unroll
    for (int a = 0; a < 3; a++)
#pragma unroll
      for (int l = 0; l < 4; l++) { bmin[a][l] = root.bmin[a][l]; bmax[a][l] = root.bmax[a][l]; }
#pragma unroll
    for (int l = 0; l < 4; l++) child[l] = root.child[l];
  }
  if (threadIdx.x < 4) cam_ctr[threadIdx.x] = 0;
  {
    const uint32_t *src = reinterpret_cast<const uint32_t *>(MatTable<DRV>::of(P));
    const uint32_t words = (P.n_materials < (uint32_t)kPipeMatMax ? P.n_materials : (uint32_t)kPipeMatMax) * (uint32_t)kMatDwords;
    for (uint32_t w = threadIdx.x; w < words; w += kBlock) mat_lds[w] = src[w];
  }
  const typename MatTable<DRV>::Rec *mats = reinterpret_cast<const typename MatTable<DRV>::Rec *>(mat_lds);
  uint32_t *lds_nodes = cam_lds;
  uint32_t *stk = cam_lds + kCamWindow * kLdsNodeStride + threadIdx.x;
  uint32_t n_lds_pk;
  const uint32_t n_lds = stage_nodes(P.scene, lds_nodes, kCamWindow, n_lds_pk);
  sobol_tables_init(sobol_tab);
  const bool defer_all = (mode & 1u) != 0;
  const uint32_t want_stack = mode >> 8;
  const uint32_t pstack = (want_stack == 0 || want_stack > (uint32_t)kCamStack) ? (uint32_t)kCamStack : want_stack;
  const size_t total = (size_t)P.n_act * n_samples;
  const size_t seg0 = (size_t)blockIdx.x * kBins * P.seg_cap;
  const V3 cam_o = ld3(P.camera.origin) + splat(0.0f);
  uint32_t n_escaped = 0, n_vertices = 0;
  for (size_t k0 = 0; k0 < P.seg_cap; k0 += kBlock) {
    if (camera_slot_sample(k0) >= total) break;
    const size_t g = camera_slot_sample(k0 + threadIdx.x);
    CameraSample cs;
    cs.o = splat(0.0f); cs.d = splat(0.0f); cs.time = 0.0f; cs.pattern = 0; cs.pix = 0; cs.sl = 0;
    int res = CAM_MISS;
    bool valid = false, alive = false;
    VertexOut v;
    v.origin = splat(0.0f); v.dir = splat(0.0f); v.beta = splat(1.0f); v.L = splat(0.0f); v.delta = false;
    if (g < total) {
      cs = camera_sample(P, g, sample_begin, sobol_tab);
      valid = true;
      bool keep = true;
      if (cull) keep = node_touched(bmin, bmax, child, cs.o.x, cs.o.y, cs.o.z, cs.d.x, cs.d.y, cs.d.z, 0.001f, CRT_INF);
      float t = 0.0f;
      uint32_t prim = kInvalid;
      if (keep)
        res = defer_all ? (int)CAM_DEFER
                        : camera_trace(P.scene, lds_nodes, n_lds, n_lds_pk, stk, kBlock, pstack, 0.001f, CRT_INF, CRT_MASK_CAMERA,
                                       cam_o.x, cam_o.y, cam_o.z, cs.d.x, cs.d.y, cs.d.z, t, prim);
      const uint32_t sl = cs.sl & 0xffffu;
      if (res == CAM_HIT) {
        float4 h;
        uint32_t gw;
        camera_hit_record(P.scene, prim, t, cs.d.x, cs.d.y, cs.d.z, h, gw);
        HitRec rec;
        rec.front_face = ((gw >> 31) & 1u) != 0;
        rec.t = h.x;
        rec.normal = v3(h.y, h.z, h.w);
        rec.p = cam_o + cs.d * rec.t;
        const auto mat = MatTable<DRV>::view(mats, P, gw & 0x7fffffffu);
        v = vertex_simple(mat, cam_o, cs.d, splat(1.0f), splat(0.0f), rec, cs.pattern, P.sample_begin + sl, 0u, (int)P.max_depth, false,
                          sobol_tab);
        alive = v.alive;
        n_vertices++;
        if (!alive) st_nt(&staging[sl * P.n_act + cs.pix], make_float4(v.L.x, v.L.y, v.L.z, 0.0f));
      } else if (res == CAM_MISS) {
        const V3 L = escaped_to_sky(cs.d, splat(1.0f), splat(0.0f));
        st_nt(&staging[sl * P.n_act + cs.pix], make_float4(L.x, L.y, L.z, 0.0f));
        n_escaped++;
      }
    }
    const size_t j = seg0 + seg_append(alive, &cam_ctr[2]);
    if (alive) {
      const uint32_t sl = cs.sl & 0xffffu;
      st_nt(&N.a[j], make_float4(v.origin.x, v.origin.y, v.origin.z, v.dir.x));
      st_nt(&N.b[j], make_float4(v.dir.y, v.dir.z, v.beta.x, v.beta.y));
      if (slim_out) {
        st_nt(&N.c[j], make_float4(v.beta.z, __uint_as_float(cs.pattern), __uint_as_float(cs.pix | (v.delta ? 0x80000000u : 0u)), __uint_as_float(sl)));
      } else {
        st_nt(&N.c[j], make_float4(v.beta.z, v.L.x, v.L.y, v.L.z));
        st_nt(&N.d[j], make_uint4(cs.pattern, cs.pix, 1u | (((P.max_depth & 0xffffu) - 1u) << 16), sl | kPrevValid | (v.delta ? kPrevDelta : 0u)));
      }
    }
    const bool later = valid && res == CAM_DEFER;
    const size_t i = seg0 + seg_append(later, &cam_ctr[0]);
    if (later) {
      st_nt(&S.a[i], make_float4(cs.d.x, cs.d.y, cs.d.z, __uint_as_float(cs.pattern)));
      st_nt(&S.d[i], make_uint4(cs.pattern, cs.pix, (P.max_depth & 0xffffu) << 16, cs.sl));
    }
  }
  add_stat(&cam_ctr[1], n_escaped);
  add_stat(&cam_ctr[3], n_vertices);
  __syncthreads();
  if (threadIdx.x == 0) {
    for (int b = 0; b < kBins; b++) {
      C->seg[0][blockIdx.x * kBins + b] = b == 0 ? cam_ctr[0] : 0;
      C->seg[1][blockIdx.x * kBins + b] = b == 0 ? cam_ctr[2] : 0;
    }
    C->shadow[blockIdx.x] = 0;
    C->cam_defer[blockIdx.x] = 0;
    if (blockIdx.x == 0) atomicAdd(&C->stats[0], (unsigned long long)total);
    const uint32_t esc = cam_ctr[1], hit = cam_ctr[3];
    if (esc + hit) atomicAdd(&C->stats[1], (unsigned long long)(esc + hit));
    if (hit) atomicAdd(&C->stats[3], (unsigned long long)hit);
    if (esc) atomicAdd(&C->stats[6], (unsigned long long)esc);
  }
}

template <bool STATS, int WIDE, int CURVE = 0>
__device__ __forceinline__ void shadow_segment(const Params &P, const PathSoA &N, const ShadowSoA &Q, Counters *C,
                                               float4 *staging, CrtTravStats *tstats, uint32_t *engine_lds) {
  const uint32_t n = ((const volatile uint32_t *)C->shadow)[blockIdx.x];
  if (n == 0) return;
  __shared__ uint32_t next;
  if (threadIdx.x == 0) next = 0;
  const uint32_t seg0 = blockIdx.x * P.seg_cap;
  LaneStats st = {};
  uint32_t err = 0, done = 0;
  auto fetch = [&](bool want, RayIn &in) -> bool {
    uint32_t k;
    if (!lds_take(want, &next, n, k)) return false;
    const uint32_t q = seg0 + k;
    const float4 A = Q.a[q], B = Q.b[q];
    in.ox = A.x; in.oy = A.y; in.oz = A.z; in.dx = B.x; in.dy = B.y; in.dz = B.z;
    in.time = B.w; in.mask = CRT_MASK_SHADOW; in.t_min = 0.001f; in.t_max = A.w; in.slot = q;
    return true;
  };
  auto emit = [&](uint32_t q, bool occ, const Hit &, float, float, float) {
    done++;
    if (occ) return;
    const float4 Cc = Q.c[q];
    const uint32_t tg = __float_as_uint(Cc.w);
    if (tg & kFilmTarget) {
      const uint32_t f = tg & ~kFilmTarget;
      float4 v = staging[f];
      v.x = v.x + Cc.x; v.y = v.y + Cc.y; v.z = v.z + Cc.z;
      staging[f] = v;
    } else {
      float4 v = N.c[tg];
      v.y = v.y + Cc.x; v.z = v.z + Cc.y; v.w = v.w + Cc.z;
      N.c[tg] = v;
    }
  };
  run_traversal<true, STATS, WIDE, (int)kColdAll | CURVE, WIDE != 0>(P.scene, engine_lds, 0.001f, err, st, fetch, emit, CRT_MASK_SHADOW);
  if (err) atomicOr(&C->err, err);
  if (STATS) flush_stats(st, tstats, done);
}
template <bool STATS, int WIDE>
__global__ __launch_bounds__(kBlock, WIDE ? 4 : CRT_SHADOW_WAVES) void k_shadow(Params P, PathSoA N, ShadowSoA Q, Counters *C,
                                                                     float4 *staging, CrtTravStats *tstats) {
  __shared__ __attribute__((aligned(16))) uint32_t engine_lds[WIDE ? kEngineLdsWide : kEngineLdsDwords];
  shadow_segment<STATS, WIDE>(P, N, Q, C, staging, tstats, engine_lds);
}
template <bool STATS>
__global__ __launch_bounds__(kBlock, CRT_SHADOW_WAVES) void k_shadow_curve(Params P, PathSoA N, ShadowSoA Q, Counters *C,
                                                                        float4 *staging, CrtTravStats *tstats) {
  __shared__ __attribute__((aligned(16))) uint32_t engine_lds[kEngineLdsDwords];
  shadow_segment<STATS, 0, (int)kColdCurve>(P, N, Q, C, staging, tstats, engine_lds);
}
template <bool STATS>
__global__ __launch_bounds__(kBlock, CRT_SHADOW_WAVES) void k_shadow_cubic(Params P, PathSoA N, ShadowSoA Q, Counters *C,
                                                                        float4 *staging, CrtTravStats *tstats) {
  __shared__ __attribute__((aligned(16))) uint32_t engine_lds[kEngineLdsDwords];
  shadow_segment<STATS, 0, (int)(kColdCurve | kColdCubic)>(P, N, Q, C, staging, tstats, engine_lds);
}

template <int MATS, bool LIT, int COLD, bool DRV>
__global__ __launch_bounds__(kBlock, CRT_EXTEND_WAVES) void k_path(Params P, PathSoA S0, PathSoA S1, HitSoA H, ShadowSoA Q, Counters *C,
                                                 float4 *staging, uint32_t sample_begin, uint32_t n_samples,
                                                 uint32_t start_it, int cur0) {
  __shared__ __attribute__((aligned(16))) uint32_t arena[kArenaDwords];
  __shared__ uint32_t live;
  if (start_it == 0) {
    generate_segment(P, S0, C, sample_begin, n_samples, arena, true);
    __syncthreads();
  }
  int cur = cur0;
  for (uint32_t it = start_it; it <= P.max_depth; it++) {
    const PathSoA &S = cur ? S1 : S0;
    const PathSoA &N = cur ? S0 : S1;
    extend_segment<false, false, COLD, false>(P, S, H, C, cur, it == 0 ? 1 : 0, nullptr, arena);
    __syncthreads();
    shade_segment<MATS, false, LIT, kArenaDwords, DRV>(P, S, N, H, Q, C, cur, staging, arena, false);
    __syncthreads();
    if (LIT) {
      shadow_segment<false, false, COLD & (int)(kColdCurve | kColdCubic)>(P, N, Q, C, staging, nullptr, arena);
      __syncthreads();
    }
    cur = 1 - cur;
    if (threadIdx.x == 0) {
      uint32_t n = 0;
      for (int b = 0; b < kBins; b++) n += ((const volatile uint32_t *)C->seg[cur])[blockIdx.x * kBins + b];
      live = n;
    }
    __syncthreads();
    if (live == 0) break;
  }
}

__global__ __launch_bounds__(kBlock) void k_resolve(const float4 *staging, uint32_t n_pix, uint32_t n_samples,
                                                    float4 *film ) {
  for (uint32_t p = blockIdx.x * kBlock + threadIdx.x; p < n_pix; p += gridDim.x * kBlock) {
    float4 acc = film[p];
    for (uint32_t s = 0; s < n_samples; s++) {
      const float4 v = staging[(size_t)s * n_pix + p];
      acc.x = acc.x + v.x; acc.y = acc.y + v.y; acc.z = acc.z + v.z;
      acc.w = acc.w + 1.0f;
    }
    film[p] = acc;
  }
}

struct PixelStats { double lum_sum, lum_sq; };
__global__ __launch_bounds__(kBlock) void k_resolve_adaptive(const float4 *staging, const uint32_t *active, uint32_t n_act,
                                                             uint32_t n_samples, float4 *film, PixelStats *stats,
                                                             uint32_t *state ,
                                                             uint32_t min_spp, float variance_threshold) {
  const double threshold = (double)variance_threshold;
  for (uint32_t a = blockIdx.x * kBlock + threadIdx.x; a < n_act; a += gridDim.x * kBlock) {
    const uint32_t p = active ? active[a] : a;
    float4 acc = film[p];
    PixelStats ps = stats[p];
    uint32_t st = state[p];
    uint32_t taken = st & 0x7fffffffu;
    bool stopped = (st >> 31) != 0;
    for (uint32_t s = 0; s < n_samples && !stopped; s++) {
      const float4 v = staging[(size_t)s * n_act + a];
      acc.x = acc.x + v.x; acc.y = acc.y + v.y; acc.z = acc.z + v.z;
      acc.w = acc.w + 1.0f;
      const double lum = (double)(0.2126f * v.x + 0.7152f * v.y + 0.0722f * v.z);
      ps.lum_sum += lum;
      ps.lum_sq += lum * lum;
      taken++;
      if (threshold > 0.0 && taken >= min_spp && taken % 4 == 0) {
        const double n = (double)taken;
        double var_of_mean = (ps.lum_sq - ps.lum_sum * ps.lum_sum / n) / (n - 1.0) / n;
        if (!(var_of_mean > 0.0)) var_of_mean = 0.0;
        double mean = ps.lum_sum / n;
        if (!(mean > 1e-4)) mean = 1e-4;
        if (sqrt(var_of_mean) / mean < threshold) stopped = true;
      }
    }
    film[p] = acc;
    stats[p] = ps;
    state[p] = taken | (stopped ? 0x80000000u : 0u);
  }
}
__global__ __launch_bounds__(kBlock) void k_compact_active(const uint32_t *state, uint32_t n_pix, uint32_t *active,
                                                           uint32_t *count) {
  for (uint32_t base = blockIdx.x * kBlock; base < n_pix; base += gridDim.x * kBlock) {
    const uint32_t p = base + threadIdx.x;
    const bool on = p < n_pix && (state[p] >> 31) == 0;
    const unsigned long long m = __ballot(on);
    if (m == 0) continue;
    const int lane = threadIdx.x & 63;
    const int leader = __ffsll((long long)m) - 1;
    uint32_t at = 0;
    if (lane == leader) at = atomicAdd(count, (uint32_t)__popcll(m));
    at = __shfl(at, leader, 64) + (uint32_t)__popcll(m & ((1ull << lane) - 1ull));
    if (on) active[at] = p;
  }
}

__global__ __launch_bounds__(kBlock) void k_film_out(const float4 *film, uint32_t n_pix, float *rgb) {
  for (uint32_t p = blockIdx.x * kBlock + threadIdx.x; p < n_pix; p += gridDim.x * kBlock) {
    const float4 v = film[p];
    rgb[3 * (size_t)p] = v.x / v.w; rgb[3 * (size_t)p + 1] = v.y / v.w; rgb[3 * (size_t)p + 2] = v.z / v.w;
  }
}

}

using ExtendFn = void (*)(Params, PathSoA, HitSoA, Counters *, int, int, CrtTravStats *);
using ExtendDeferredFn = void (*)(Params, PathSoA, HitSoA, Counters *, int, int, CrtTravStats *, const uint32_t *);
using PathFn = void (*)(Params, PathSoA, PathSoA, HitSoA, ShadowSoA, Counters *, float4 *, uint32_t, uint32_t, uint32_t, int);
using ShadeFn = void (*)(Params, PathSoA, PathSoA, HitSoA, ShadowSoA, Counters *, int, float4 *, int);
using ShadePipeFn = void (*)(Params, PathSoA, PathSoA, HitSoA, Counters *, int, float4 *, int, uint32_t, int);
using CameraVertexFn = void (*)(Params, PathSoA, PathSoA, Counters *, uint32_t, uint32_t, float4 *, uint32_t, int);
using ShadowFn = void (*)(Params, PathSoA, ShadowSoA, Counters *, float4 *, CrtTravStats *);
using ShadeVolFn = void (*)(Params, PathSoA, PathSoA, HitSoA, ShadowSoA, Counters *, int, float4 *, int, uint32_t *);
template <class Fn>
struct InstanceRow { InstanceKey key; Fn fn; };
#define CRT_ROW(family, kernel, ...) {CRT_INSTANCE_KEY(family, kernel, __VA_ARGS__), kernel<__VA_ARGS__>},
static const InstanceRow<ExtendFn> kExtendRows[] = {CRT_INSTANCES_EXTEND(CRT_ROW)};
static const InstanceRow<ExtendDeferredFn> kExtendDeferredRows[] = {CRT_INSTANCES_EXTEND_DEFERRED(CRT_ROW)};
static const InstanceRow<PathFn> kPathRows[] = {CRT_INSTANCES_PATH(CRT_ROW)};
static const InstanceRow<ShadeFn> kShadeRows[] = {CRT_INSTANCES_SHADE(CRT_ROW)};
static const InstanceRow<ShadePipeFn> kShadePipeRows[] = {CRT_INSTANCES_SHADE_PIPE(CRT_ROW) CRT_INSTANCES_SHADE_PIPE_SLIM(CRT_ROW)};
static const InstanceRow<ShadowFn> kShadowRows[] = {CRT_INSTANCES_SHADOW(CRT_ROW)};
static const InstanceRow<ShadeVolFn> kShadeVolRows[] = {CRT_INSTANCES_SHADE_VOL(CRT_ROW)};
#undef CRT_ROW
template <class Fn, size_t N>
static bool find_instance(const InstanceRow<Fn> (&rows)[N], const InstanceKey &key, Fn &fn) {
  fn = nullptr;
  if (key.none()) return true;
  for (const InstanceRow<Fn> &r : rows)
    if (r.key == key) { fn = r.fn; return true; }
  set_error_text("render refused: no such instance in this build (family %d: %d, %d, %d, %d, %d)", (int)key.family, (int)key.arg[0],
                 (int)key.arg[1], (int)key.arg[2], (int)key.arg[3], (int)key.arg[4]);
  return false;
}

struct Renderer {
  std::shared_ptr<Scene> scene;
  Params P{};
  std::vector<uint32_t> pixels;
  struct Lane {
    size_t cap_slots = 0;
    char *blob = nullptr;
    size_t blob_bytes = 0;
    PathSoA S[2]{};
    HitSoA H{};
    ShadowSoA Q{};
    uint32_t *qseed = nullptr;
    Counters *C = nullptr;
    float4 *staging = nullptr;
    hipStream_t stream = nullptr;
    hipEvent_t done = nullptr;
  };
  static constexpr int kMaxLanes = 4;
  Lane lanes[kMaxLanes];
  int n_lanes = 4;
  int last_lanes = 1;
  size_t lane_min_paths = (size_t)96 << 20;
  hipEvent_t ev_start = nullptr;
  float4 *film = nullptr;
  CrtMaterial *d_materials = nullptr;
  DevMaterial *d_mat_derived = nullptr;
  uint8_t *d_mat_class = nullptr;
  uint16_t *d_mat_index = nullptr;
  DevMedium *d_media = nullptr;
  bool has_media = false;
  PixelStats *d_pstats = nullptr;
  uint32_t *d_state = nullptr, *d_active = nullptr, *d_count = nullptr;
  uint32_t n_act = 0, min_spp = 2;
  float variance_threshold = 0.0f;
  PlanInputs in;
  LaunchPlan last_plan;
  CrtVolumes *volumes = nullptr;
  VolArgs vol{nullptr, nullptr, 0};
  void estimate_root_miss_share() {
    in.root_miss_share = 0.0f;
    if (!scene || scene->bvh.wide.empty()) return;
    const WideNode &nd = scene->bvh.wide[0];
    uint32_t child[4];
    for (int l = 0; l < 4; l++) child[l] = (nd.flags & (1u << l)) ? 0u : kInvalid;
    const CrtCamera &c = P.camera;
    constexpr int GW = 32, GH = 18;
    int missed = 0;
    for (int j = 0; j < GH; j++)
      for (int i = 0; i < GW; i++) {
        const float sx = ((float)i + 0.5f) / (float)GW, sy = ((float)j + 0.5f) / (float)GH;
        float d[3];
        for (int a = 0; a < 3; a++) d[a] = c.lower_left[a] + c.horizontal[a] * sx + c.vertical[a] * sy - c.origin[a];
        if (!node_touched(nd.bmin, nd.bmax, child, c.origin[0], c.origin[1], c.origin[2], d[0], d[1], d[2], 0.001f, CRT_INF)) missed++;
      }
    in.root_miss_share = (float)missed / (float)(GW * GH);
  }
  size_t max_batch_slots = 0;
  int cus = 256, fused_mult = 3, stage_mult = 8, mult_forced = 0;
  CrtLight *d_lights = nullptr;
  std::vector<std::shared_ptr<void>> environments;
  uint32_t *d_pixels = nullptr;
  int grid = 768;
  hipStream_t last_stream = nullptr;
  bool profile = false;
  struct Ev { hipEvent_t a, b; int cls; };
  std::vector<Ev> events;
  double prof_ms[4] = {0, 0, 0, 0};
  uint64_t prof_launches[4] = {0, 0, 0, 0};

  ~Renderer() {
    drain_events();
    for (Lane &B : lanes) {
      if (B.stream) (void)hipStreamSynchronize(B.stream);
      if (B.blob) (void)hipFree(B.blob);
      if (B.C) (void)hipFree(B.C);
      if (B.stream) (void)hipStreamDestroy(B.stream);
      if (B.done) (void)hipEventDestroy(B.done);
    }
    if (ev_start) (void)hipEventDestroy(ev_start);
    volumes_release(volumes);
    if (film) (void)hipFree(film);
    if (d_materials) (void)hipFree(d_materials);
    if (d_mat_derived) (void)hipFree(d_mat_derived);
    if (d_mat_class) (void)hipFree(d_mat_class);
    if (d_mat_index) (void)hipFree(d_mat_index);
    if (d_media) (void)hipFree(d_media);
    if (d_pstats) (void)hipFree(d_pstats);
    if (d_state) (void)hipFree(d_state);
    if (d_active) (void)hipFree(d_active);
    if (d_count) (void)hipFree(d_count);
    if (d_lights) (void)hipFree(d_lights);
    if (d_pixels) (void)hipFree(d_pixels);
  }

  void drain_events() {
    for (Ev &e : events) {
      float ms = 0.0f;
      if (hipEventSynchronize(e.b) == hipSuccess && hipEventElapsedTime(&ms, e.a, e.b) == hipSuccess) {
        prof_ms[e.cls] += ms;
        prof_launches[e.cls]++;
      }
      (void)hipEventDestroy(e.a);
      (void)hipEventDestroy(e.b);
    }
    events.clear();
  }

  int batch_grid(size_t total, bool fused_pipeline) const {
    int mult = fused_pipeline ? fused_mult : stage_mult;
    if (!mult_forced)
      while (mult < 64 && total / ((size_t)cus * mult) > ((size_t)192 << 10)) mult *= 2;
    const int g = cus * mult;
    return g > kMaxGrid ? kMaxGrid : g;
  }

  int ensure_buffers(Lane &B, size_t slots) {
    size_t &cap_slots = B.cap_slots, &blob_bytes = B.blob_bytes;
    char *&blob = B.blob;
    PathSoA (&S)[2] = B.S;
    HitSoA &H = B.H;
    ShadowSoA &Q = B.Q;
    float4 *&staging = B.staging;
    if (slots <= cap_slots && blob && !(last_lanes > 1 && cap_slots > slots + slots / 2)) return CRT_OK;
    if (blob) { (void)hipFree(blob); blob = nullptr; }
    const size_t total = slots, cap = slots;
    const size_t bcap = cap * kBins;
    if (total == 0 || bcap >= (size_t)0x7fffffff) return CRT_ERR_BAD_ARG;
    const size_t p16 = (cap * 16 + 255) & ~size_t(255);
    const size_t b16 = (bcap * 16 + 255) & ~size_t(255), b4 = (bcap * 4 + 255) & ~size_t(255);
    const bool lit = P.n_lights > 0, motion = P.has_motion != 0;
    const size_t p4 = (lit && volumes) ? ((cap * 4 + 255) & ~size_t(255)) : 0;
    blob_bytes = 2 * ((lit ? 5 : 4) * b16 + (motion ? b4 : 0)) + (b16 + b4) + (lit ? 3 * p16 : 0) + p4 + p16;
    const size_t want_bytes = (max_batch_slots && slots > max_batch_slots) ? ((size_t)1 << 46) : blob_bytes;
    if (!CRT_HIP_OK(hipMalloc(&blob, want_bytes))) {
      (void)hipGetLastError();
      blob = nullptr; blob_bytes = 0; cap_slots = 0;
      return CRT_ERR_NO_DEVICE;
    }
    char *cur_p = blob;
    auto take = [&](size_t bytes) { char *r = cur_p; cur_p += bytes; return r; };
    for (int b = 0; b < 2; b++) {
      S[b].a = (float4 *)take(b16); S[b].b = (float4 *)take(b16); S[b].c = (float4 *)take(b16);
      S[b].d = (uint4 *)take(b16);
      S[b].e = lit ? (float4 *)take(b16) : nullptr;
      S[b].time = motion ? (float *)take(b4) : nullptr;
    }
    H.h = (float4 *)take(b16); H.geom = (uint32_t *)take(b4);
    if (lit) { Q.a = (float4 *)take(p16); Q.b = (float4 *)take(p16); Q.c = (float4 *)take(p16); }
    B.qseed = p4 ? (uint32_t *)take(p4) : nullptr;
    staging = (float4 *)take(p16);
    cap_slots = cap;
    return CRT_OK;
  }

  template <class F>
  void timed(int cls, hipStream_t st, F &&launch) {
    if (!profile) { launch(); return; }
    Ev e; e.cls = cls;
    (void)hipEventCreate(&e.a); (void)hipEventCreate(&e.b);
    (void)hipEventRecord(e.a, st);
    launch();
    (void)hipEventRecord(e.b, st);
    events.push_back(e);
  }

  int render(uint32_t sample_begin, uint32_t n_samples, hipStream_t st, CrtTravStats *d_tstats) {
    if (n_samples == 0) return CRT_OK;
    if (n_samples > 0xffffu) return CRT_ERR_BAD_ARG;
    (void)hipGetLastError();
    last_stream = st;
    int L = n_lanes;
    const size_t total = (size_t)P.n_pix * n_samples;
    if (d_tstats || variance_threshold > 0.0f) L = 1;
    while (L > 1 && (total / L < lane_min_paths || n_samples < (uint32_t)L)) L--;
    last_lanes = L < 1 ? 1 : L;
    for (int l = L < 1 ? 1 : L; l < kMaxLanes; l++) {
      Lane &B = lanes[l];
      if (!B.blob) continue;
      if (B.stream) (void)hipStreamSynchronize(B.stream);
      (void)hipFree(B.blob);
      B.blob = nullptr; B.cap_slots = 0; B.blob_bytes = 0;
    }
    if (L <= 1) return render_lane(lanes[0], sample_begin, n_samples, st, d_tstats, true);
    if (!ev_start && !CRT_HIP_OK(hipEventCreateWithFlags(&ev_start, hipEventDisableTiming))) return CRT_ERR_NO_DEVICE;
    for (int l = 1; l < L; l++) {
      Lane &B = lanes[l];
      if (!B.stream && !CRT_HIP_OK(hipStreamCreateWithFlags(&B.stream, hipStreamNonBlocking))) return CRT_ERR_NO_DEVICE;
      if (!B.done && !CRT_HIP_OK(hipEventCreateWithFlags(&B.done, hipEventDisableTiming))) return CRT_ERR_NO_DEVICE;
    }
    uint32_t begin[kMaxLanes], count[kMaxLanes];
    for (int l = 0; l < L; l++) {
      count[l] = n_samples / L + ((uint32_t)l < n_samples % L ? 1u : 0u);
      begin[l] = l == 0 ? sample_begin : begin[l - 1] + count[l - 1];
    }
    for (int l = 0; l < L; l++) {
      Params scratch = P;
      const int rc = plan_lane(lanes[l], scratch, count[l], false);
      if (rc != CRT_OK) return rc;
    }
    if (!CRT_HIP_OK(hipEventRecord(ev_start, st))) return CRT_ERR_NO_DEVICE;
    auto fail = [&](int rc) {
      for (int l = 1; l < L; l++)
        if (lanes[l].stream) (void)hipStreamSynchronize(lanes[l].stream);
      (void)hipStreamSynchronize(st);
      return rc;
    };
    for (int l = L - 1; l >= 0; l--) {
      hipStream_t ls = l == 0 ? st : lanes[l].stream;
      if (l > 0 && !CRT_HIP_OK(hipStreamWaitEvent(ls, ev_start, 0))) return fail(CRT_ERR_NO_DEVICE);
      const int rc = render_lane(lanes[l], begin[l], count[l], ls, nullptr, false);
      if (rc != CRT_OK) return fail(rc);
      if (l > 0 && !CRT_HIP_OK(hipEventRecord(lanes[l].done, ls))) return fail(CRT_ERR_NO_DEVICE);
    }
    for (int l = 0; l < L; l++) {
      if (l > 0 && !CRT_HIP_OK(hipStreamWaitEvent(st, lanes[l].done, 0))) return fail(CRT_ERR_NO_DEVICE);
      timed(3, st, [&] { hipLaunchKernelGGL(k_resolve, dim3(grid), dim3(kBlock), 0, st, lanes[l].staging, P.n_pix, count[l], film); });
    }
    return CRT_HIP_OK(hipGetLastError()) ? CRT_OK : fail(CRT_ERR_NO_DEVICE);
  }

  int plan_lane(Lane &B, Params &p, uint32_t n_samples, bool stats) {
    const size_t total = (size_t)p.n_act * n_samples;
    in.total = total;
    in.stats = stats;
    in.scene = P.scene;
    in.n_lights = P.n_lights; in.has_inf_lights = P.has_inf_lights != 0; in.has_env = P.envs != nullptr; in.strategy = P.strategy;
    in.has_motion = P.has_motion != 0; in.lens = P.camera.lens_radius > 0.0f;
    in.mat_index = P.mat_index != nullptr; in.partition = P.partition; in.n_materials = P.n_materials; in.max_depth = P.max_depth;
    in.class_stats = P.class_stats;
    in.volumes = volumes != nullptr;
    in.partial_active = p.active != nullptr;
    if (in.volumes && stats) {
      set_error_text("render refused: the stats build does not run volume renders");
      return CRT_ERR_UNSUPPORTED;
    }
    if (plan_launches(in, last_plan) != CRT_OK) {
      set_error_text("render refused: the selected kernels (wide %d, cold %d / %d) cannot run this image (direct words %u, cold %u)",
                     (int)last_plan.wide, last_plan.ext_cold, last_plan.path_cold, P.scene.direct_leaves, P.scene.cold);
      return CRT_ERR_UNSUPPORTED;
    }
    grid = batch_grid(total, last_plan.fused);
    p.seg_cap = (uint32_t)(((total + (size_t)grid * kBlock - 1) / ((size_t)grid * kBlock)) * kBlock);
    p.cam_compact = last_plan.cam_compact;
    p.root_cull = last_plan.root_cull ? 1u : 0u;
    if (const int rc = ensure_buffers(B, (size_t)p.seg_cap * grid)) return rc;
    if (last_plan.slim_state && p.n_act > 0x7fffffffu) {
      set_error_text("render refused: %u active pixels do not fit the slim path state's 31 bits", p.n_act);
      return CRT_ERR_BAD_ARG;
    }
    return CRT_OK;
  }

  int render_lane(Lane &B, uint32_t sample_begin, uint32_t n_samples, hipStream_t st, CrtTravStats *d_tstats, bool fold_here) {
    PathSoA (&S)[2] = B.S;
    HitSoA &H = B.H;
    ShadowSoA &Q = B.Q;
    Counters *C = B.C;
    const bool adaptive = variance_threshold > 0.0f;
    if (adaptive && n_act == 0) return CRT_OK;
    Params p = P;
    p.sample_begin = sample_begin;
    p.n_act = adaptive ? n_act : P.n_pix;
    p.active = (adaptive && n_act < P.n_pix) ? d_active : nullptr;
    if (const int rc = plan_lane(B, p, n_samples, d_tstats != nullptr)) return rc;
    const LaunchPlan plan = last_plan;
    PathFn path;
    ExtendFn extend;
    ExtendDeferredFn extend_deferred;
    ShadeFn shade;
    ShadePipeFn shade_pipe, shade_slim;
    ShadowFn shadow;
    ShadeVolFn shade_vol = nullptr;
    if (plan.volumes && !find_instance(kShadeVolRows, plan.shade, shade_vol)) return CRT_ERR_UNSUPPORTED;
    if (plan.volumes != (volumes != nullptr) || (plan.volumes && (plan.volume_key.none() || plan.fused))) return CRT_ERR_UNSUPPORTED;
    if (!find_instance(kPathRows, plan.path, path) || !find_instance(kExtendRows, plan.extend, extend) ||
        (!plan.volumes && !find_instance(kShadeRows, plan.shade, shade)) || !find_instance(kShadePipeRows, plan.shade_early, shade_pipe) ||
        !find_instance(kShadePipeRows, plan.shade_slim_key(), shade_slim) ||
        !find_instance(kShadowRows, plan.shadow_key, shadow) ||
        !find_instance(kExtendDeferredRows, plan.extend_deferred_key(), extend_deferred))
      return CRT_ERR_UNSUPPORTED;
    if (plan.camera_trace && (!extend_deferred || plan.cam_compact == 0 || plan.fused)) return CRT_ERR_UNSUPPORTED;
    float4 *staging = B.staging;
    auto fold = [&]() -> int {
      if (!fold_here) return CRT_HIP_OK(hipGetLastError()) ? CRT_OK : CRT_ERR_NO_DEVICE;
      if (!adaptive) {
        timed(3, st, [&] { hipLaunchKernelGGL(k_resolve, dim3(grid), dim3(kBlock), 0, st, staging, P.n_pix, n_samples, film); });
        return CRT_HIP_OK(hipGetLastError()) ? CRT_OK : CRT_ERR_NO_DEVICE;
      }
      timed(3, st, [&] {
        hipLaunchKernelGGL(k_resolve_adaptive, dim3(grid), dim3(kBlock), 0, st, staging, p.active, p.n_act, n_samples, film,
                           d_pstats, d_state, min_spp, variance_threshold);
        (void)hipMemsetAsync(d_count, 0, 4, st);
        hipLaunchKernelGGL(k_compact_active, dim3(grid), dim3(kBlock), 0, st, d_state, P.n_pix, d_active, d_count);
      });
      uint32_t h = 0;
      if (!CRT_HIP_OK(hipMemcpyAsync(&h, d_count, 4, hipMemcpyDeviceToHost, st)) || !CRT_HIP_OK(hipStreamSynchronize(st)))
        return CRT_ERR_NO_DEVICE;
      n_act = h;
      return CRT_OK;
    };
    if (plan.fused) {
      timed(0, st, [&] { hipLaunchKernelGGL(path, dim3(grid), dim3(kBlock), 0, st, p, S[0], S[1], H, Q, C, staging, sample_begin, n_samples, 0u, 0); });
      return fold();
    }
    Params p0 = p;
    if (plan.camera_vertex) {
      p0.cam_compact = 2;
      const uint32_t nx = 1;
      const int slim_out = (shade_slim && nx <= P.max_depth && nx < plan.tail_at && (int)nx < plan.noclassify_from) ? 1 : 0;
      const CameraVertexFn fn = plan.shade_early.arg[0] ? k_camera_vertex<true> : k_camera_vertex<false>;
      timed(3, st, [&] { hipLaunchKernelGGL(fn, dim3(grid), dim3(kBlock), 0, st, p, S[0], S[1], C, sample_begin, n_samples, staging, plan.camera_mode, slim_out); });
    } else if (plan.camera_trace)
      timed(3, st, [&] { hipLaunchKernelGGL(k_camera, dim3(grid), dim3(kBlock), 0, st, p, S[0], reinterpret_cast<uint32_t *>(S[1].a), H, C, sample_begin, n_samples, staging, plan.camera_mode); });
    else
      timed(3, st, [&] { hipLaunchKernelGGL(k_generate, dim3(grid), dim3(kBlock), 0, st, p, S[0], C, sample_begin, n_samples, staging); });
    int cur = 0;
    for (uint32_t it = 0; it <= P.max_depth; it++) {
      if (it >= plan.tail_at) {
        timed(3, st, [&] { hipLaunchKernelGGL(path, dim3(grid), dim3(kBlock), 0, st, p, S[0], S[1], H, Q, C, staging, sample_begin, n_samples, it, cur); });
        break;
      }
      const int first = it == 0 ? 1 : 0;
      if (first && plan.camera_vertex)
        timed(0, st, [&] { hipLaunchKernelGGL(extend, dim3(grid), dim3(kBlock), 0, st, p0, S[cur], H, C, cur, first, d_tstats); });
      else if (first && plan.camera_trace)
        timed(0, st, [&] { hipLaunchKernelGGL(extend_deferred, dim3(grid), dim3(kBlock), 0, st, p, S[cur], H, C, cur, first, d_tstats, reinterpret_cast<const uint32_t *>(S[1 - cur].a)); });
      else
        timed(0, st, [&] { hipLaunchKernelGGL(extend, dim3(grid), dim3(kBlock), 0, st, p, S[cur], H, C, cur, first, d_tstats); });
      if (plan.volumes) {
        timed(3, st, [&] { hipLaunchKernelGGL(k_volume, dim3(grid), dim3(kBlock), 0, st, p, S[cur], H, C, cur, first, vol); });
        timed(1, st, [&] { hipLaunchKernelGGL(shade_vol, dim3(grid), dim3(kBlock), 0, st, p, S[cur], S[1 - cur], H, Q, C, cur, staging, (int)it >= plan.noclassify_from ? 2 : 0, B.qseed); });
        if (!plan.shadow_volume_key.none())
          timed(3, st, [&] { hipLaunchKernelGGL(k_shadow_volume, dim3(grid), dim3(kBlock), 0, st, p, Q, (const uint32_t *)B.qseed, C, vol); });
      } else if (shade_pipe && (int)it < plan.noclassify_from) {
        const uint32_t nx = it + 1;
        const int out_full = (nx <= P.max_depth && nx < plan.tail_at && (int)nx < plan.noclassify_from) ? 0 : 1;
        const ShadePipeFn fn = shade_slim ? shade_slim : shade_pipe;
        if (first && plan.camera_vertex)
          timed(1, st, [&] { hipLaunchKernelGGL(fn, dim3(grid), dim3(kBlock), 0, st, p0, S[cur], S[1 - cur], H, C, cur, staging, first | 2, it, out_full); });
        else
          timed(1, st, [&] { hipLaunchKernelGGL(fn, dim3(grid), dim3(kBlock), 0, st, p, S[cur], S[1 - cur], H, C, cur, staging, first, it, out_full); });
      } else
        timed(1, st, [&] { hipLaunchKernelGGL(shade, dim3(grid), dim3(kBlock), 0, st, p, S[cur], S[1 - cur], H, Q, C, cur, staging, first | ((int)it >= plan.noclassify_from ? 2 : 0)); });
      if (shadow)
        timed(2, st, [&] { hipLaunchKernelGGL(shadow, dim3(grid), dim3(kBlock), 0, st, p, S[1 - cur], Q, C, staging, d_tstats ? d_tstats + 1 : nullptr); });
      cur = 1 - cur;
    }
    return fold();
  }
};

}

struct CrtRenderer { crt::Renderer r; };

using namespace crt;

extern "C" {

void crt_camera_new(CrtCamera *c, const float lookfrom[3], const float lookat[3], const float vup[3], float vfov_deg,
                    float aspect, float aperture, float focus_dist) {
  if (!c) return;
  auto sub = [](const float a[3], const float b[3], float o[3]) { for (int i = 0; i < 3; i++) o[i] = a[i] - b[i]; };
  auto nrm = [](float a[3]) {
    const float l = sqrtf((a[0] * a[0] + a[1] * a[1]) + a[2] * a[2]);
    for (int i = 0; i < 3; i++) a[i] = a[i] / l;
  };
  auto crs = [](const float a[3], const float b[3], float o[3]) {
    o[0] = a[1] * b[2] - b[1] * a[2]; o[1] = a[2] * b[0] - b[2] * a[0]; o[2] = a[0] * b[1] - b[0] * a[1];
  };
  const float theta = vfov_deg * 3.14159265358979323846f / 180.0f;
  const float h = tanf(theta / 2.0f);
  const float viewport_height = 2.0f * h;
  const float viewport_width = aspect * viewport_height;
  float w[3], u[3], v[3];
  sub(lookfrom, lookat, w); nrm(w);
  crs(vup, w, u); nrm(u);
  crs(w, u, v);
  for (int i = 0; i < 3; i++) {
    c->origin[i] = lookfrom[i];
    c->horizontal[i] = u[i] * (focus_dist * viewport_width);
    c->vertical[i] = v[i] * (focus_dist * viewport_height);
    c->lower_left[i] = ((lookfrom[i] - c->horizontal[i] / 2.0f) - c->vertical[i] / 2.0f) - w[i] * focus_dist;
    c->u[i] = u[i];
    c->v[i] = v[i];
  }
  c->lens_radius = aperture / 2.0f;
}

static CrtRenderer *renderer_new(CrtScene *scene, const CrtMaterial *materials, size_t n_materials, const CrtLight *lights,
                                 size_t n_lights, const CrtCamera *camera, const CrtRenderSettings *settings,
                                 uint32_t tile_rank, uint32_t tile_world) {
  if (!scene || !camera || !settings || (n_materials && !materials) || (n_lights && !lights)) return nullptr;
  if (tile_world == 0 || tile_rank >= tile_world) return nullptr;
  if (!(settings->variance_threshold >= 0.0f)) return nullptr;
  if (n_materials < scene->p->n_geoms) return nullptr;
  if (settings->max_depth > 0xffffu) return nullptr;
  if (scene->p->ensure_device() != CRT_OK) return nullptr;
  CrtRenderer *R = new (std::nothrow) CrtRenderer();
  if (!R) return nullptr;
  struct Hold { CrtRenderer *p; ~Hold() { delete p; } } hold{R};
  const Knobs knobs = read_knobs();
  Renderer &r = R->r;
  r.scene = scene->p;
  Params &P = r.P;
  P.scene = scene->p->dev->view;
  P.n_lights = (uint32_t)n_lights;
  P.n_materials = (uint32_t)n_materials;
  P.has_inf_lights = 0;
  for (size_t k = 0; k < n_lights; k++) {
    if (lights[k].kind > CRT_LIGHT_DOME_MAP) { set_error_text("crt_renderer_new: light %zu has the unknown kind %u", k, lights[k].kind); return nullptr; }
    if (lights[k].kind >= CRT_LIGHT_DISTANT) P.has_inf_lights = 1;
    if (lights[k].kind == CRT_LIGHT_DOME_MAP) {
      uint32_t id;
      std::memcpy(&id, &lights[k].center[0], 4);
      std::shared_ptr<void> env = env_retain(id);
      if (!env) { set_error_text("crt_renderer_new: light %zu names environment id 0x%x, which is not live", k, id); return nullptr; }
      r.environments.push_back(std::move(env));
    }
  }
  P.envs = nullptr;
  if (!r.environments.empty()) {
    const void *table = nullptr;
    if (env_table_for_launch(&table) != CRT_OK || !table) return nullptr;
    P.envs = static_cast<const EnvSlot *>(table);
  }
  P.camera = *camera;
  P.width = settings->width; P.height = settings->height; P.max_depth = settings->max_depth;
  P.frame = settings->frame; P.strategy = settings->strategy; P.filter_kind = settings->filter_kind;
  P.filter_radius = settings->filter_radius;
  P.has_motion = scene->p->has_motion ? 1u : 0u;
  r.pixels.resize(crt_shard_pixels(P.width, P.height, tile_rank, tile_world, nullptr));
  crt_shard_pixels(P.width, P.height, tile_rank, tile_world, r.pixels.data());
  P.n_pix = (uint32_t)r.pixels.size();
  P.n_act = P.n_pix; P.active = nullptr;
  r.variance_threshold = settings->variance_threshold;
  r.min_spp = settings->min_spp > 2 ? settings->min_spp : 2;
  r.n_act = P.n_pix;
  bool ok = P.n_pix > 0;
  if (ok && r.variance_threshold > 0.0f) {
    ok = CRT_HIP_OK(hipMalloc(&r.d_pstats, (size_t)P.n_pix * sizeof(PixelStats))) &&
         CRT_HIP_OK(hipMemset(r.d_pstats, 0, (size_t)P.n_pix * sizeof(PixelStats))) &&
         CRT_HIP_OK(hipMalloc(&r.d_state, (size_t)P.n_pix * 4)) && CRT_HIP_OK(hipMemset(r.d_state, 0, (size_t)P.n_pix * 4)) &&
         CRT_HIP_OK(hipMalloc(&r.d_active, (size_t)P.n_pix * 4)) && CRT_HIP_OK(hipMalloc(&r.d_count, 4));
  }
  for (Renderer::Lane &B : r.lanes)
    ok = ok && CRT_HIP_OK(hipMalloc(&B.C, sizeof(Counters))) && CRT_HIP_OK(hipMemset(B.C, 0, sizeof(Counters)));
  ok = ok && CRT_HIP_OK(hipMalloc(&r.film, (size_t)P.n_pix * 16)) && CRT_HIP_OK(hipMemset(r.film, 0, (size_t)P.n_pix * 16));
  ok = ok && CRT_HIP_OK(hipMalloc(&r.d_pixels, (size_t)P.n_pix * 4)) &&
       CRT_HIP_OK(hipMemcpy(r.d_pixels, r.pixels.data(), (size_t)P.n_pix * 4, hipMemcpyHostToDevice));
  std::vector<CrtMaterial> unique_mats;
  std::vector<uint16_t> mat_index;
  {
    bool dedup = CRT_MAT_INDEX_BUILD && n_materials > (size_t)mat_lds_max(kArenaDwords);
    dedup = dedup && knobs.mat_dedup != 0;
    if (dedup) {
      auto bytes_of = [](const CrtMaterial &m) { return std::string(reinterpret_cast<const char *>(&m), sizeof(CrtMaterial)); };
      std::unordered_map<std::string, uint32_t> seen;
      mat_index.resize(n_materials);
      for (size_t k = 0; k < n_materials && dedup; k++) {
        auto it = seen.emplace(bytes_of(materials[k]), (uint32_t)unique_mats.size());
        if (it.second) unique_mats.push_back(materials[k]);
        if (unique_mats.size() > 0xffffu) dedup = false;
        mat_index[k] = (uint16_t)it.first->second;
      }
      if (!dedup || unique_mats.size() == n_materials) { unique_mats.clear(); mat_index.clear(); }
    }
  }
  if (!unique_mats.empty()) {
    ok = ok && CRT_HIP_OK(hipMalloc(&r.d_mat_index, n_materials * sizeof(uint16_t))) &&
         CRT_HIP_OK(hipMemcpy(r.d_mat_index, mat_index.data(), n_materials * sizeof(uint16_t), hipMemcpyHostToDevice));
    materials = unique_mats.data();
    n_materials = unique_mats.size();
    P.n_materials = (uint32_t)n_materials;
  }
  P.mat_index = r.d_mat_index;
  if (ok && n_materials) {
    ok = CRT_HIP_OK(hipMalloc(&r.d_materials, n_materials * sizeof(CrtMaterial))) &&
         CRT_HIP_OK(hipMemcpy(r.d_materials, materials, n_materials * sizeof(CrtMaterial), hipMemcpyHostToDevice));
  }
  if (ok && n_materials) {
    ok = CRT_HIP_OK(hipMalloc(&r.d_mat_derived, n_materials * sizeof(DevMaterial)));
    if (ok) {
      hipLaunchKernelGGL(k_derive_materials, dim3((unsigned)((n_materials + 255) / 256)), dim3(256), 0, nullptr, r.d_materials,
                         (uint32_t)n_materials, r.d_mat_derived);
      ok = CRT_HIP_OK(hipGetLastError());
    }
  }
  if (ok && n_materials) {
    std::vector<uint8_t> cls(n_materials);
    bool seen[kClasses] = {false, false, false, false};
    for (size_t k = 0; k < n_materials; k++) { cls[k] = material_class(materials[k]); seen[cls[k]] = true; }
    int distinct = 0;
    for (int c = 0; c < kClasses; c++) distinct += seen[c] ? 1 : 0;
    P.partition = distinct > 1 ? 1u : 0u;
    if (knobs.partition >= 0) P.partition = knobs.partition ? 1u : 0u;
    ok = CRT_HIP_OK(hipMalloc(&r.d_mat_class, n_materials)) &&
         CRT_HIP_OK(hipMemcpy(r.d_mat_class, cls.data(), n_materials, hipMemcpyHostToDevice));
  }
  if (ok && n_lights) {
    ok = CRT_HIP_OK(hipMalloc(&r.d_lights, n_lights * sizeof(CrtLight))) &&
         CRT_HIP_OK(hipMemcpy(r.d_lights, lights, n_lights * sizeof(CrtLight), hipMemcpyHostToDevice));
  }
  if (ok && n_materials) {
    uint32_t *d_count = nullptr, h_count = 0;
    ok = CRT_HIP_OK(hipMalloc(&r.d_media, 2 * n_materials * sizeof(DevMedium))) && CRT_HIP_OK(hipMalloc(&d_count, 4));
    if (ok) {
      hipLaunchKernelGGL(k_build_media, dim3((unsigned)((n_materials + 255) / 256)), dim3(256), 0, nullptr, r.d_materials,
                         (uint32_t)n_materials, r.d_media);
      hipLaunchKernelGGL(k_number_media, dim3(1), dim3(kNumberBlock), 0, nullptr, (uint32_t)n_materials, r.d_media,
                         r.d_media + n_materials, d_count);
      ok = CRT_HIP_OK(hipGetLastError()) && CRT_HIP_OK(hipMemcpy(&h_count, d_count, 4, hipMemcpyDeviceToHost));
      ok = ok && h_count <= kMaxMedia;
      r.has_media = h_count > 0;
    }
    if (d_count) (void)hipFree(d_count);
  }
  if (!ok) return nullptr;
  {
    bool simple = true;
    for (size_t k = 0; k < n_materials; k++) simple = simple && material_class(materials[k]) <= 1;
    simple = simple && knobs.simple != 0;
    r.in.mats_kind = r.has_media ? 2 : (simple ? 0 : 1);
    if ((P.scene.cold & kColdCurve) && r.in.mats_kind == 0) r.in.mats_kind = 1;
  }
  P.materials = r.d_materials; P.mat_derived = r.d_mat_derived; P.lights = r.d_lights; P.pixel_index = r.d_pixels;
  P.mat_class = r.d_mat_class;
  P.media = r.d_media; P.media_by_id = r.d_media ? r.d_media + n_materials : nullptr;
  hipDeviceProp_t prop;
  int dev = 0;
  (void)hipGetDevice(&dev);
  if (select_engine_env(P.scene, r.in.engine, true) != CRT_OK) {
    set_error_text("crt_renderer_new: no traversal-engine instance of this build can decode the scene image");
    return nullptr;
  }
  PlanInputs &in = r.in;
  in.cam_compact_build = CRT_CAM_COMPACT_BUILD != 0; in.shade_pipe_build = kShadePipeBuild; in.root_cull_build = kRootCullBuild;
  in.pipe_mat_max = kPipeMatMax;
  in.prefer_stage = knobs.prefer_stage != 0;
  in.cam_compact_ok = knobs.cam_compact != 0;
  in.root_cull_knob = knobs.root_cull;
  r.estimate_root_miss_share();
  in.noclassify_from = knobs.noclassify_from;
  in.shade_pipe = knobs.shade_pipe;
  in.slim_state = knobs.slim_state;
  in.camera_trace_knob = knobs.camera_trace;
  in.camera_vertex_knob = knobs.camera_vertex;
  in.camera_trace_build = kRootCullBuild && CRT_CAM_COMPACT_BUILD != 0;
  in.no_emitter = table_has_no_emitter(materials, n_materials);
  in.mat_derived = knobs.mat_derived != 0;
  in.tail_from = knobs.tail_from;
  in.shade_wide = knobs.shade_wide;
  in.force_fused = knobs.fused;
  in.stage_min_paths = knobs.stage_min_paths;
  r.max_batch_slots = knobs.max_batch_slots;
  r.n_lanes = knobs.lanes < 1 ? 1 : (knobs.lanes > Renderer::kMaxLanes ? Renderer::kMaxLanes : knobs.lanes);
  r.lane_min_paths = knobs.lane_min_paths;
  if (hipGetDeviceProperties(&prop, dev) == hipSuccess && prop.multiProcessorCount > 0) r.cus = prop.multiProcessorCount;
  r.stage_mult = in.engine.wide ? 8 : 3;
  if (knobs.grid_mult > 0) { r.fused_mult = r.stage_mult = knobs.grid_mult; r.mult_forced = 1; }
  r.last_plan.fused = in.force_fused >= 0 ? in.force_fused != 0 : !in.prefer_stage;
  r.last_plan.wide = !r.last_plan.fused && in.engine.wide;
  r.grid = r.batch_grid(0, r.last_plan.fused);
  hold.p = nullptr;
  return R;
}
CrtRenderer *crt_renderer_new(CrtScene *scene, const CrtMaterial *materials, size_t n_materials, const CrtLight *lights,
                              size_t n_lights, const CrtCamera *camera, const CrtRenderSettings *settings,
                              uint32_t tile_rank, uint32_t tile_world) {
  CrtRenderer *R = nullptr;
  (void)abi_guard("crt_renderer_new", [&] {
    R = renderer_new(scene, materials, n_materials, lights, n_lights, camera, settings, tile_rank, tile_world);
    return (int)CRT_OK;
  });
  return R;
}
void crt_renderer_free(CrtRenderer *r) { delete r; }
size_t crt_renderer_pixel_count(const CrtRenderer *r) { return r ? r->r.pixels.size() : 0; }
int crt_renderer_pixel_indices(const CrtRenderer *r, uint32_t *out) {
  if (!r || !out) return CRT_ERR_BAD_ARG;
  std::memcpy(out, r->r.pixels.data(), r->r.pixels.size() * 4);
  return CRT_OK;
}
int crt_render_samples(CrtRenderer *r, uint32_t sample_begin, uint32_t sample_count, void *stream) {
  if (!r) return CRT_ERR_BAD_ARG;
  return abi_guard("crt_render_samples", [&] { return r->r.render(sample_begin, sample_count, (hipStream_t)stream, nullptr); });
}
constexpr bool kVolumeRenderBuild = !kRegenFirst;
static int renderer_set_volumes(CrtRenderer *r, CrtVolumes *v) {
  Renderer &R = r->r;
  if (v == R.volumes) return CRT_OK;
  if (v && !kVolumeRenderBuild) {
    set_error_text("crt_renderer_set_volumes: a CRT_REGEN_FIRST build holds no volume stage");
    return CRT_ERR_UNSUPPORTED;
  }
  VolumesView view;
  if (v) {
    const int rc = volumes_device(v, view);
    if (rc != CRT_OK) return rc;
  }
  if (!CRT_HIP_OK(hipStreamSynchronize(R.last_stream))) return CRT_ERR_NO_DEVICE;
  for (Renderer::Lane &B : R.lanes) {
    if (B.stream) (void)hipStreamSynchronize(B.stream);
    if (B.blob) (void)hipFree(B.blob);
    B.blob = nullptr; B.cap_slots = 0; B.blob_bytes = 0; B.qseed = nullptr;
  }
  volumes_retain(v);
  volumes_release(R.volumes);
  R.volumes = v;
  R.vol = VolArgs{view.regions, view.grid, view.n_regions};
  return CRT_OK;
}
int crt_renderer_set_volumes(CrtRenderer *r, CrtVolumes *v) {
  if (!r) return CRT_ERR_BAD_ARG;
  return abi_guard("crt_renderer_set_volumes", [&] { return renderer_set_volumes(r, v); });
}
int crt_render_samples_stats(CrtRenderer *r, uint32_t sample_begin, uint32_t sample_count, void *stream,
                             CrtTravStats host_stats[2]) {
  if (!r || !host_stats) return CRT_ERR_BAD_ARG;
  if (r->r.volumes) { set_error_text("crt_render_samples_stats: the stats build does not run volume renders"); return CRT_ERR_UNSUPPORTED; }
  CrtTravStats *d = nullptr;
  if (!CRT_HIP_OK(hipMalloc(&d, 2 * sizeof(CrtTravStats)))) return CRT_ERR_NO_DEVICE;
  (void)hipMemsetAsync(d, 0, 2 * sizeof(CrtTravStats), (hipStream_t)stream);
  int rc = abi_guard("crt_render_samples_stats", [&] { return r->r.render(sample_begin, sample_count, (hipStream_t)stream, d); });
  CrtTravStats h[2] = {};
  if (rc == CRT_OK && !CRT_HIP_OK(hipMemcpyAsync(h, d, sizeof h, hipMemcpyDeviceToHost, (hipStream_t)stream))) rc = CRT_ERR_NO_DEVICE;
  if (!CRT_HIP_OK(hipStreamSynchronize((hipStream_t)stream))) rc = CRT_ERR_NO_DEVICE;
  (void)hipFree(d);
  if (rc == CRT_OK) {
    for (int w = 0; w < 2; w++) {
      for (int k = 0; k < 2; k++) {
        host_stats[w].queries[k] += h[w].queries[k]; host_stats[w].nodes[k] += h[w].nodes[k];
        host_stats[w].leaves[k] += h[w].leaves[k]; host_stats[w].packets[k] += h[w].packets[k];
        host_stats[w].prims[k] += h[w].prims[k];
      }
      host_stats[w].accepted_hits += h[w].accepted_hits; host_stats[w].instance_descents += h[w].instance_descents;
      host_stats[w].rays += h[w].rays;
      for (int k = 0; k < 8; k++) { host_stats[w].phase_waves[k] += h[w].phase_waves[k]; host_stats[w].phase_lanes[k] += h[w].phase_lanes[k]; host_stats[w].phase_cycles[k] += h[w].phase_cycles[k]; }
    }
  }
  return rc;
}
int crt_film_resolve(CrtRenderer *r, float *d_rgb, void *stream) {
  if (!r || !d_rgb) return CRT_ERR_BAD_ARG;
  hipLaunchKernelGGL(k_film_out, dim3(r->r.grid), dim3(kBlock), 0, (hipStream_t)stream, r->r.film, r->r.P.n_pix, d_rgb);
  return CRT_HIP_OK(hipGetLastError()) ? CRT_OK : CRT_ERR_NO_DEVICE;
}
int crt_film_read(CrtRenderer *r, float *host_rgb) {
  if (!r || !host_rgb) return CRT_ERR_BAD_ARG;
  float *d = nullptr;
  const size_t bytes = (size_t)r->r.P.n_pix * 12;
  if (!CRT_HIP_OK(hipMalloc(&d, bytes))) return CRT_ERR_NO_DEVICE;
  int rc = crt_film_resolve(r, d, r->r.last_stream);
  if (rc == CRT_OK && !CRT_HIP_OK(hipStreamSynchronize(r->r.last_stream))) rc = CRT_ERR_NO_DEVICE;
  if (rc == CRT_OK && !CRT_HIP_OK(hipMemcpy(host_rgb, d, bytes, hipMemcpyDeviceToHost))) rc = CRT_ERR_NO_DEVICE;
  (void)hipFree(d);
  return rc;
}
int crt_film_clear(CrtRenderer *r, void *stream) {
  if (!r) return CRT_ERR_BAD_ARG;
  bool ok = CRT_HIP_OK(hipMemsetAsync(r->r.film, 0, (size_t)r->r.P.n_pix * 16, (hipStream_t)stream));
  for (Renderer::Lane &B : r->r.lanes) ok = ok && CRT_HIP_OK(hipMemsetAsync(B.C, 0, sizeof(Counters), (hipStream_t)stream));
  if (ok && r->r.d_state) {
    ok = CRT_HIP_OK(hipMemsetAsync(r->r.d_state, 0, (size_t)r->r.P.n_pix * 4, (hipStream_t)stream)) &&
         CRT_HIP_OK(hipMemsetAsync(r->r.d_pstats, 0, (size_t)r->r.P.n_pix * sizeof(PixelStats), (hipStream_t)stream));
    r->r.n_act = r->r.P.n_pix;
  }
  return ok ? CRT_OK : CRT_ERR_NO_DEVICE;
}
int crt_render_stats(CrtRenderer *r, CrtRayStats *out) {
  if (!r || !out) return CRT_ERR_BAD_ARG;
  struct { uint32_t err, pad; unsigned long long stats[8]; } h;
  static_assert(offsetof(Counters, seg) == sizeof h, "Counters head layout");
  if (!CRT_HIP_OK(hipStreamSynchronize(r->r.last_stream))) return CRT_ERR_NO_DEVICE;
  unsigned long long sum[8] = {0, 0, 0, 0, 0, 0, 0, 0};
  uint32_t err = 0;
  for (const Renderer::Lane &B : r->r.lanes) {
    if (!CRT_HIP_OK(hipMemcpy(&h, B.C, sizeof h, hipMemcpyDeviceToHost))) return CRT_ERR_NO_DEVICE;
    for (int k = 0; k < 8; k++) sum[k] += h.stats[k];
    err |= h.err;
  }
  out->camera_rays = sum[0]; out->closest_hit = sum[1]; out->shadow_rays = sum[2];
  out->vertices = sum[3]; out->rr_tested = sum[4]; out->rr_killed = sum[5];
  out->ended_escaped = sum[6]; out->ended_depth = sum[7];
  return err ? CRT_ERR_STACK : CRT_OK;
}
size_t crt_renderer_active_pixels(const CrtRenderer *r) { return r ? (r->r.variance_threshold > 0.0f ? r->r.n_act : r->r.P.n_pix) : 0; }
int crt_renderer_sample_counts(CrtRenderer *r, uint32_t *host_out) {
  if (!r || !host_out) return CRT_ERR_BAD_ARG;
  if (!r->r.d_state) return CRT_ERR_UNSUPPORTED;
  if (!CRT_HIP_OK(hipStreamSynchronize(r->r.last_stream))) return CRT_ERR_NO_DEVICE;
  if (!CRT_HIP_OK(hipMemcpy(host_out, r->r.d_state, (size_t)r->r.P.n_pix * 4, hipMemcpyDeviceToHost))) return CRT_ERR_NO_DEVICE;
  for (size_t k = 0; k < r->r.P.n_pix; k++) host_out[k] &= 0x7fffffffu;
  return CRT_OK;
}
int crt_renderer_shade_class_stats(CrtRenderer *r, int enable, uint64_t out_waves[4], uint64_t out_lanes[4]) {
  if (!r) return CRT_ERR_BAD_ARG;
  Renderer &R = r->r;
  if (out_waves && out_lanes) {
    unsigned long long h[8];
    if (!CRT_HIP_OK(hipStreamSynchronize(R.last_stream))) return CRT_ERR_NO_DEVICE;
    for (int c = 0; c < 4; c++) out_waves[c] = out_lanes[c] = 0;
    for (Renderer::Lane &B : R.lanes) {
      if (!CRT_HIP_OK(hipMemcpy(h, B.C->cls_waves, sizeof h, hipMemcpyDeviceToHost))) return CRT_ERR_NO_DEVICE;
      if (!CRT_HIP_OK(hipMemset(B.C->cls_waves, 0, sizeof h))) return CRT_ERR_NO_DEVICE;
      for (int c = 0; c < 4; c++) { out_waves[c] += h[c]; out_lanes[c] += h[4 + c]; }
    }
  }
  if (enable >= 0) R.P.class_stats = enable ? 1u : 0u;
  return CRT_OK;
}
int crt_renderer_lanes(const CrtRenderer *r) { return r ? r->r.last_lanes : 0; }
int crt_renderer_set_lanes(CrtRenderer *r, int lanes) {
  if (!r) return CRT_ERR_BAD_ARG;
  r->r.n_lanes = lanes < 1 ? 1 : (lanes > Renderer::kMaxLanes ? Renderer::kMaxLanes : lanes);
  return r->r.n_lanes;
}
int crt_renderer_pipeline(const CrtRenderer *r, uint32_t out[3]) {
  if (!r || !out) return CRT_ERR_BAD_ARG;
  const LaunchPlan &plan = r->r.last_plan;
  out[0] = plan.fused ? 1u : 0u;
  out[1] = (plan.wide ? 1u : 0u) | (plan.shade_piped() ? 2u : 0u) | (plan.root_cull ? 4u : 0u) | (plan.slim_state ? 8u : 0u) |
           (plan.volumes ? 16u : 0u) | (plan.camera_trace ? 32u : 0u) | (plan.camera_vertex ? 64u : 0u);
  out[2] = (uint32_t)r->r.grid;
  return CRT_OK;
}
int crt_renderer_profile(CrtRenderer *r, int enable) {
  if (!r) return CRT_ERR_BAD_ARG;
  r->r.drain_events();
  r->r.profile = enable != 0;
  for (int k = 0; k < 4; k++) { r->r.prof_ms[k] = 0; r->r.prof_launches[k] = 0; }
  return CRT_OK;
}
int crt_renderer_profile_read(CrtRenderer *r, double out_ms[4], uint64_t out_launches[4]) {
  if (!r || !out_ms || !out_launches) return CRT_ERR_BAD_ARG;
  r->r.drain_events();
  for (int k = 0; k < 4; k++) { out_ms[k] = r->r.prof_ms[k]; out_launches[k] = r->r.prof_launches[k]; }
  return CRT_OK;
}

}
```

crust-render_amd/csrc/kernels/qmc.hip.h:

```cpp
#pragma once

#include <hip/hip_runtime.h>

namespace crt {
namespace dev {

struct Sampler { uint32_t pattern, index; };

__device__ const uint32_t kSobolDirs[4][32] = {
    {0x80000000u, 0x40000000u, 0x20000000u, 0x10000000u, 0x08000000u, 0x04000000u, 0x02000000u, 0x01000000u,
     0x00800000u, 0x00400000u, 0x00200000u, 0x00100000u, 0x00080000u, 0x00040000u, 0x00020000u, 0x00010000u,
     0x00008000u, 0x00004000u, 0x00002000u, 0x00001000u, 0x00000800u, 0x00000400u, 0x00000200u, 0x00000100u,
     0x00000080u, 0x00000040u, 0x00000020u, 0x00000010u, 0x00000008u, 0x00000004u, 0x00000002u, 0x00000001u},
    {0x80000000u, 0xc0000000u, 0xa0000000u, 0xf0000000u, 0x88000000u, 0xcc000000u, 0xaa000000u, 0xff000000u,
     0x80800000u, 0xc0c00000u, 0xa0a00000u, 0xf0f00000u, 0x88880000u, 0xcccc0000u, 0xaaaa0000u, 0xffff0000u,
     0x80008000u, 0xc000c000u, 0xa000a000u, 0xf000f000u, 0x88008800u, 0xcc00cc00u, 0xaa00aa00u, 0xff00ff00u,
     0x80808080u, 0xc0c0c0c0u, 0xa0a0a0a0u, 0xf0f0f0f0u, 0x88888888u, 0xccccccccu, 0xaaaaaaaau, 0xffffffffu},
    {0x80000000u, 0xc0000000u, 0x60000000u, 0x90000000u, 0xe8000000u, 0x5c000000u, 0x8e000000u, 0xc5000000u,
     0x68800000u, 0x9cc00000u, 0xee600000u, 0x55900000u, 0x80680000u, 0xc09c0000u, 0x60ee0000u, 0x90550000u,
     0xe8808000u, 0x5cc0c000u, 0x8e606000u, 0xc5909000u, 0x6868e800u, 0x9c9c5c00u, 0xeeee8e00u, 0x5555c500u,
     0x8000e880u, 0xc0005cc0u, 0x60008e60u, 0x9000c590u, 0xe8006868u, 0x5c009c9cu, 0x8e00eeeeu, 0xc5005555u},
    {0x80000000u, 0xc0000000u, 0x20000000u, 0x50000000u, 0xf8000000u, 0x74000000u, 0xa2000000u, 0x93000000u,
     0xd8800000u, 0x25400000u, 0x59e00000u, 0xe6d00000u, 0x78080000u, 0xb40c0000u, 0x82020000u, 0xc3050000u,
     0x208f8000u, 0x51474000u, 0xfbea2000u, 0x75d93000u, 0xa0858800u, 0x914e5400u, 0xdbe79e00u, 0x25db6d00u,
     0x58800080u, 0xe54000c0u, 0x79e00020u, 0xb6d00050u, 0x800800f8u, 0xc00c0074u, 0x200200a2u, 0x50050093u}};

__device__ __forceinline__ uint32_t pcg_hash(uint32_t v) {
  const uint32_t state = v * 747796405u + 2891336453u;
  const uint32_t word = ((state >> ((state >> 28u) + 4u)) ^ state) * 277803737u;
  return (word >> 22u) ^ word;
}
__device__ __forceinline__ uint32_t laine_karras(uint32_t x, uint32_t seed) {
  x ^= x * 0x3d20adeau;
  x += seed;
  x *= (seed >> 16) | 1u;
  x ^= x * 0x05526c56u;
  x ^= x * 0x53a22864u;
  return x;
}
__device__ __forceinline__ uint32_t owen(uint32_t x, uint32_t seed) {
  return __brev(laine_karras(__brev(x), seed));
}
__device__ __forceinline__ float unit_f32(uint32_t x) { return (float)(x >> 8) * (1.0f / 16777216.0f); }

__device__ __forceinline__ Sampler sampler_new(int x, int y, int frame, int index) {
  const uint32_t pixel = ((uint32_t)x & 0xffu) | (((uint32_t)y & 0xffu) << 8);
  return Sampler{pcg_hash(pcg_hash((uint32_t)frame) ^ pixel), (uint32_t)index};
}
__device__ __forceinline__ Sampler new_domain(Sampler s, int key) {
  return Sampler{pcg_hash(s.pattern + 0x9e3779b9u * ((uint32_t)key + 1u)), s.index};
}
constexpr int kSobolLdsWords = 3 * 4 * 256;

__device__ __forceinline__ void sobol_tables_init(uint32_t *tab ) {
  for (int e = threadIdx.x; e < kSobolLdsWords; e += blockDim.x) {
    const int v = e & 255, k = (e >> 8) & 3, d = (e >> 10) + 1;
    uint32_t x = 0;
#pragma unroll
    for (int b = 0; b < 8; b++)
      if ((v >> b) & 1) x ^= kSobolDirs[d][8 * k + b];
    tab[e] = x;
  }
  __syncthreads();
}

__device__ __forceinline__ void draw_sample4(Sampler s, float out[4], const uint32_t *tab) {
  const uint32_t idx = owen(s.index, pcg_hash(s.pattern));
  const uint32_t b0 = idx & 255u, b1 = (idx >> 8) & 255u, b2 = (idx >> 16) & 255u, b3 = idx >> 24;
#pragma unroll
  for (int d = 0; d < 4; d++) {
    uint32_t x;
    if (d == 0) {
      x = __brev(idx);
    } else {
      const uint32_t *t = tab + (d - 1) * 1024;
      x = t[b0] ^ t[256 + b1] ^ t[512 + b2] ^ t[768 + b3];
    }
    x = owen(x, pcg_hash(s.pattern + (uint32_t)d + 1u));
    out[d] = unit_f32(x);
  }
}
__device__ __forceinline__ float draw_rnd1(Sampler s) {
  return unit_f32(pcg_hash(s.pattern ^ (s.index * 0x9e3779b9u + 0x7f4a7c15u)));
}
__device__ __forceinline__ uint32_t rng_seed(Sampler s) { return s.pattern ^ (s.index * 0x9e3779b9u + 0x7f4a7c15u); }

}
}
```

crust-render_amd/csrc/scene.cpp:

```cpp
#include <hip/hip_runtime.h>

#include <cstdarg>
#include <cstdio>
#include <cmath>
#include <cstring>
#include <algorithm>
#include <utility>
#include <unordered_map>

#include <cstdlib>
#include "crt_internal.h"

namespace crt {

static F3 mat3_mul(const Mat3 &m, F3 r) {
  F3 res = m.x * r.x;
  res = res + m.y * r.y;
  res = res + m.z * r.z;
  return res;
}
Mat3 mat3_transpose(const Mat3 &m) {
  return {f3(m.x.x, m.y.x, m.z.x), f3(m.x.y, m.y.y, m.z.y), f3(m.x.z, m.y.z, m.z.z)};
}
static Mat3 mat3_inverse(const Mat3 &m) {
// ... 48 lines not shown
          Prim p{};
          p.kind = PRIM_TRI;
          p.geom_id = geom_id;
          p.prim_id = uint32_t(t);
          p.mask = g.mask;
          p.v0 = vert(g.verts, i0);
          p.v1 = vert(g.verts, i1);
          p.v2 = vert(g.verts, i2);
          if (g.has_normals && i0 < nn && i1 < nn && i2 < nn) {
            p.has_normals = true;
            p.n0 = vert(g.normals, i0);
            p.n1 = vert(g.normals, i1);
            p.n2 = vert(g.normals, i2);
          }
          prims.push_back(std::move(p));
        }
        break;
      }
      case G_SPHERE: {
        Prim p{};
        p.kind = PRIM_SPHERE;
        p.geom_id = geom_id;
        p.mask = g.mask;
        p.center = g.center;
        p.radius = g.radius;
        prims.push_back(std::move(p));
        break;
      }
      case G_CURVES: {
        const size_t ns = g.segs.size() / 8;
        for (size_t k = 0; k < ns; k++) {
          const float *sg = &g.segs[8 * k];
          Prim p{};
          p.kind = PRIM_CURVE;
          p.geom_id = geom_id;
          p.prim_id = uint32_t(k);
          p.mask = g.mask;
          p.v0 = f3(sg[0], sg[1], sg[2]);
          p.radius = sg[3];
          p.v1 = f3(sg[4], sg[5], sg[6]);
          p.radius1 = sg[7];
          prims.push_back(std::move(p));
        }
        break;
      }
      case G_CUBICS: {
        const size_t ns = g.segs.size() / 14;
        for (size_t k = 0; k < ns; k++) {
          const float *sp = &g.segs[14 * k];
          Prim p{};
          p.kind = PRIM_CUBIC;
          p.geom_id = geom_id;
          p.prim_id = uint32_t(k);
          p.mask = g.mask;
          p.v0 = f3(sp[0], sp[1], sp[2]);
          p.v1 = f3(sp[3], sp[4], sp[5]);
          p.v2 = f3(sp[6], sp[7], sp[8]);
          p.v3 = f3(sp[9], sp[10], sp[11]);
          p.radius = sp[12];
          p.radius1 = sp[13];
          p.depth = cubic_flatness_depth(sp, 2.0f * (sp[12] > sp[13] ? sp[12] : sp[13]));
          prims.push_back(std::move(p));
        }
        break;
      }
      case G_INSTANCE: {
        if (!g.scene || !g.scene->bvh.has_bbox) break;
        const Aabb inner = g.scene->bvh.root_bbox;
        Prim p{};
        p.kind = PRIM_INSTANCE;
        p.geom_id = geom_id;
        p.mask = g.mask;
        p.scene = g.scene;
        p.l2w = g.l2w;
        p.w2l = affine_inverse(g.l2w);
        p.normal_mat = mat3_transpose(Mat3{p.w2l.x, p.w2l.y, p.w2l.z});
        p.has_end = g.has_end;
        p.l2w_end = g.l2w_end;
        if (g.has_end) {
          Aabb a = transformed_aabb(inner, g.l2w), e = transformed_aabb(inner, g.l2w_end);
          p.bounds = Aabb{vmin(a.mn, e.mn), vmax(a.mx, e.mx)};
        } else {
          p.bounds = transformed_aabb(inner, g.l2w);
        }
        has_motion |= g.has_end || g.scene->has_motion;
        if (g.scene->depth + 1 > depth) depth = g.scene->depth + 1;
        prims.push_back(std::move(p));
        break;
      }
    }
  }
  if (depth > kMaxInstanceLevels) {
    set_error_text("commit: %u levels of instance nesting, the kernels carry %u", depth, kMaxInstanceLevels);
    return nullptr;
  }
  scene->depth = depth;
  scene->has_motion = has_motion;
  build_bvh(scene->bvh, std::move(prims));
  return scene;
}

DeviceImage::~DeviceImage() {
  if (blob) (void)hipFree(blob);
}

static thread_local char g_last_error[512] = "";
const char *last_error_text() { return g_last_error; }
bool hip_failed(int err, const char *what, const char *file, int line) {
  if (err == (int)hipSuccess) return false;
  std::snprintf(g_last_error, sizeof g_last_error, "%s -> %s (%d) at %s:%d", what, hipGetErrorString((hipError_t)err), err,
                file, line);
  return true;
}

void set_error_text(const char *fmt, ...) {
  va_list ap;
  va_start(ap, fmt);
  std::vsnprintf(g_last_error, sizeof g_last_error, fmt, ap);
  va_end(ap);
}

Knobs read_knobs() {
  Knobs k;
  auto num = [](const char *name, long long &out) {
    const char *e = getenv(name);
    if (!e || !*e) return false;
    char *end = nullptr;
    const long long v = strtoll(e, &end, 10);
    if (end == e) return false;
    out = v;
    return true;
  };
  long long v;
  if (num("CRT_POOL_STACK_RT", v)) k.pool_stack_deep = v >= CRT_POOL_STACK_DEEP ? 1 : 0;
  if (num("CRT_DIRECT_LEAVES", v)) k.direct_leaves = v != 0;
  if (num("CRT_DIRECT_INST", v)) k.direct_inst = v != 0;
  if (num("CRT_STAGE_ROOTS", v)) k.stage_roots = (int)std::min<long long>(std::max<long long>(v, 0), 1 << 20);
  if (num("CRT_COLD", v)) k.cold = (uint32_t)v & kColdAll;
  if (num("CRT_INST_ORDER", v)) k.inst_order = v != 0;
  if (num("CRT_HOT_PACKETS", v)) k.hot_packets = v != 0;
  if (num("CRT_WIDE", v)) k.wide = v == 2 ? 2 : (v != 0);
  if (num("CRT_MAT_DEDUP", v)) k.mat_dedup = v != 0;
  if (num("CRT_PARTITION", v)) k.partition = v != 0;
  if (num("CRT_SIMPLE", v)) k.simple = v != 0;
  if (num("CRT_PREFER_STAGE", v)) k.prefer_stage = v != 0;
  if (num("CRT_CAM_COMPACT", v)) k.cam_compact = v != 0;
  if (num("CRT_ROOT_CULL", v)) k.root_cull = v != 0 ? 1 : 0;
  if (num("CRT_SHADE_WIDE", v)) k.shade_wide = v != 0;
  if (num("CRT_SHADE_PIPE", v)) k.shade_pipe = v != 0;
  if (num("CRT_MAT_DERIVED", v)) k.mat_derived = v != 0;
  if (num("CRT_SLIM_STATE", v)) k.slim_state = v != 0;
  if (num("CRT_CAMERA_TRACE", v)) k.camera_trace = (v >= 0 && v <= 3) ? (int)v : 1;
  if (num("CRT_CAMERA_VERTEX", v)) k.camera_vertex = v != 0 ? 1 : 0;
  if (num("CRT_FUSED", v)) k.fused = v != 0;
  if (num("CRT_NOCLASSIFY_FROM", v)) k.noclassify_from = (int)std::min<long long>(std::max<long long>(v, 0), 1 << 30);
  if (num("CRT_TAIL_FROM", v)) k.tail_from = (int)std::min<long long>(std::max<long long>(v, 0), 1 << 30);
  if (num("CRT_LANES", v)) k.lanes = (int)std::min<long long>(std::max<long long>(v, 1), 4);
  if (num("CRT_GRID_MULT", v)) k.grid_mult = (int)std::min<long long>(std::max<long long>(v, 0), 64);
  if (num("CRT_MAX_BATCH_SLOTS", v)) k.max_batch_slots = v > 0 ? (size_t)v : 0;
  if (num("CRT_LANE_MIN_PATHS", v)) k.lane_min_paths = v > 0 ? (size_t)v : 1;
  if (num("CRT_STAGE_MIN_PATHS", v)) k.stage_min_paths = v > 0 ? (size_t)v : 1;
  return k;
}
int wide_request() { return read_knobs().wide; }

int device_ok() {
  static int ok = [] {
    int n = 0;
    if (!CRT_HIP_OK(hipGetDeviceCount(&n)) || n <= 0) return 0;
    return 1;
  }();
  return ok;
}

namespace {
struct Flat {
  std::vector<WideNode> nodes;
  std::vector<Leaf> leaves;
  std::vector<Tri4> packets;
  std::vector<uint32_t> indices;
  std::vector<DevPrim> prims;
  std::vector<DevInstance> instances;
  std::vector<std::pair<uint32_t, DevInstanceMotion>> moving;
  std::vector<float> normals;
  struct Placed { uint32_t root; uint32_t has_packets; };
  std::unordered_map<const Scene *, Placed> placed;
};

void put_affine(float out[12], const Affine &a) {
  const float v[12] = {a.x.x, a.x.y, a.x.z, a.y.x, a.y.y, a.y.z, a.z.x, a.z.y, a.z.z, a.t.x, a.t.y, a.t.z};
  std::memcpy(out, v, sizeof v);
}
uint32_t f2u(float f) { uint32_t u; std::memcpy(&u, &f, 4); return u; }
float u2f(uint32_t u) { float f; std::memcpy(&f, &u, 4); return f; }

Flat::Placed place(Flat &f, const Scene &s) {
  auto it = f.placed.find(&s);
  if (it != f.placed.end()) return it->second;
  const Bvh &b = s.bvh;
  std::vector<Flat::Placed> inner(b.prims.size(), Flat::Placed{CRT_INVALID_ID, 0});
  for (size_t i = 0; i < b.prims.size(); i++)
    if (b.prims[i].kind == PRIM_INSTANCE) inner[i] = place(f, *b.prims[i].scene);

  const uint32_t node0 = uint32_t(f.nodes.size()), leaf0 = uint32_t(f.leaves.size());
  const uint32_t pkt0 = uint32_t(f.packets.size()), idx0 = uint32_t(f.indices.size());
  const uint32_t prim0 = uint32_t(f.prims.size());
  std::vector<uint32_t> rec(b.prims.size());
  {
    uint32_t next = prim0;
    for (size_t i = 0; i < b.prims.size(); i++) { rec[i] = next; next += b.prims[i].kind == PRIM_CUBIC ? 2u : 1u; }
  }
  for (WideNode n : b.wide) {
    for (int l = 0; l < 4; l++) {
      if (!(n.flags & (1u << l))) continue;
      n.child[l] += (n.flags & (1u << (4 + l))) ? leaf0 : node0;
    }
    f.nodes.push_back(n);
  }
  for (Leaf l : b.leaves) {
    l.pkt_first += pkt0;
    l.idx_first += idx0;
    f.leaves.push_back(l);
  }
  for (Tri4 p : b.packets) {
    for (int l = 0; l < 4; l++)
      if (p.active & (1u << l)) p.prim[l] = rec[p.prim[l]];
    f.packets.push_back(p);
  }
  std::vector<uint32_t> inst_slot(b.prims.size(), CRT_INVALID_ID);
  {
    uint32_t next_slot = uint32_t(f.instances.size());
    if (read_knobs().inst_order)
    for (uint32_t i : b.indices)
      if (b.prims[i].kind == PRIM_INSTANCE && inst_slot[i] == CRT_INVALID_ID) inst_slot[i] = next_slot++;
    for (size_t i = 0; i < b.prims.size(); i++)
      if (b.prims[i].kind == PRIM_INSTANCE && inst_slot[i] == CRT_INVALID_ID) inst_slot[i] = next_slot++;
    f.instances.resize(next_slot);
  }
  for (size_t i = 0; i < b.prims.size(); i++) {
    const Prim &p = b.prims[i];
    DevPrim d{};
    d.kind = p.kind;
    d.geom_id = p.geom_id;
    d.prim_id = p.prim_id;
    d.mask = p.mask;
    if (p.kind == PRIM_TRI) {
      const float v[9] = {p.v0.x, p.v0.y, p.v0.z, p.v1.x, p.v1.y, p.v1.z, p.v2.x, p.v2.y, p.v2.z};
      std::memcpy(d.d, v, sizeof v);
      if (p.has_normals) {
        d.d[9] = u2f(uint32_t(f.normals.size() / 9));
        d.d[10] = u2f(kSmoothNormalTag);
        const float n[9] = {p.n0.x, p.n0.y, p.n0.z, p.n1.x, p.n1.y, p.n1.z, p.n2.x, p.n2.y, p.n2.z};
        f.normals.insert(f.normals.end(), n, n + 9);
      } else {
        flat_tri_normal(d.d, d.d + 9);
      }
    } else if (p.kind == PRIM_SPHERE) {
      d.d[0] = p.center.x; d.d[1] = p.center.y; d.d[2] = p.center.z; d.d[3] = p.radius;
    } else if (p.kind == PRIM_CURVE) {
      d.d[0] = p.v0.x; d.d[1] = p.v0.y; d.d[2] = p.v0.z; d.d[3] = p.radius;
      d.d[4] = p.v1.x; d.d[5] = p.v1.y; d.d[6] = p.v1.z; d.d[7] = p.radius1;
    } else if (p.kind == PRIM_CUBIC) {
      const float cp[12] = {p.v0.x, p.v0.y, p.v0.z, p.v1.x, p.v1.y, p.v1.z, p.v2.x, p.v2.y, p.v2.z, p.v3.x, p.v3.y, p.v3.z};
      std::memcpy(d.d, cp, sizeof cp);
      f.prims.push_back(d);
      d.kind = PRIM_CUBIC_TAIL;
      std::memset(d.d, 0, sizeof d.d);
      d.d[0] = p.radius; d.d[1] = p.radius1; d.d[2] = u2f(p.depth);
    } else {
      DevInstance in{};
      put_affine(in.w2l, p.w2l);
      in.root = inner[i].root;
      in.flags = (inner[i].has_packets ? 1u : 0u) | (p.has_end ? 2u : 0u);
      in.geom_id = p.geom_id;
      in.mask = p.mask;
      d.d[0] = u2f(inst_slot[i]);
      f.instances[inst_slot[i]] = in;
      if (p.has_end) {
        DevInstanceMotion mo{};
        put_affine(mo.l2w, p.l2w);
        put_affine(mo.l2w_end, p.l2w_end);
        f.moving.emplace_back(inst_slot[i], mo);
      }
    }
    f.prims.push_back(d);
  }
  for (uint32_t i : b.indices)
    f.indices.push_back(b.prims[i].kind == PRIM_INSTANCE ? (kIndexInstance | inst_slot[i]) : rec[i]);
  Flat::Placed me{b.wide.empty() ? CRT_INVALID_ID : node0, b.packets.empty() ? 0u : 1u};
  f.placed.emplace(&s, me);
  return me;
}
}

namespace {
struct FlatImage {
  Flat f;
  Flat::Placed me{CRT_INVALID_ID, 0};
  uint32_t pool_stack = 6;
  bool direct = false;
  std::vector<uint32_t> leaf_of_word;
  uint32_t n_staged_roots = 0;
  uint32_t n_top_packets = 0;
  uint32_t cold = kColdAll;
};

// ... 441 lines not shown
```

Baseline: 12420 Mray/s.

## Precompute per-pixel camera seeds in a table and read root cull node from LDS

```diff
diff --git a/crust-render_amd/__init__.py b/crust-render_amd/__init__.py
--- a/crust-render_amd/__init__.py
+++ b/crust-render_amd/__init__.py
@@ -853,7 +853,8 @@
         _check(lib().crt_renderer_pipeline(self.h, out), "crt_renderer_pipeline")
         return dict(fused=bool(out[0]), wide=bool(out[1] & 1), shade_pipe=bool(out[1] & 2), root_cull=bool(out[1] & 4),
                     slim_state=bool(out[1] & 8), volumes=bool(out[1] & 16), camera_trace=bool(out[1] & 32),
-                    camera_vertex=bool(out[1] & 64), grid=int(out[2]))
+                    camera_vertex=bool(out[1] & 64), pixel_table=bool(out[1] & 128), cull_root_lds=bool(out[1] & 256),
+                    grid=int(out[2]))
 
     def lanes(self):
         return int(lib().crt_renderer_lanes(self.h)) if hasattr(lib(), "crt_renderer_lanes") else 1
diff --git a/crust-render_amd/csrc/crt_internal.h b/crust-render_amd/csrc/crt_internal.h
--- a/crust-render_amd/csrc/crt_internal.h
+++ b/crust-render_amd/csrc/crt_internal.h
@@ -358,6 +358,9 @@
   int pipe_mat_max = 0;
   bool camera_trace_build = true;
   int camera_vertex_knob = -1;
+  int pixel_table_knob = -1;
+  bool pixel_table_ready = false;
+  int cull_root_lds_knob = -1;
 };
 constexpr uint32_t kCameraTraceMaxNodes = 1024;
 constexpr float kRootCullMinShare = 0.125f;
@@ -403,6 +406,8 @@
     return k;
   }
   bool camera_vertex = false;
+  bool pixel_table = false;
+  bool cull_root_lds = false;
 };
 inline EngineSelect engine_of_width(const EngineSelect &e, const DevScene &s, int w) {
   EngineSelect l = e;
@@ -464,12 +469,14 @@
                       (q.camera_trace_knob > 0 || q.scene.n_nodes <= kCameraTraceMaxNodes);
     if (pl.camera_trace) pl.camera_mode = q.camera_trace_knob == 2 ? 1u : (q.camera_trace_knob == 3 ? (1u << 8) : 0u);
     pl.camera_vertex = pl.camera_trace && pl.shade_piped() && q.max_depth >= 1 && q.camera_vertex_knob != 0;
+    pl.pixel_table = pl.camera_trace && q.pixel_table_knob != 0 && q.pixel_table_ready;
+    pl.cull_root_lds = pl.camera_trace && pl.root_cull && q.cull_root_lds_knob != 0 && q.scene.root == 0 && q.scene.n_nodes > 0;
   }
   const bool ok = !(q.volumes && q.stats) &&
                   (pl.path.none() || engine_accepts(engine_of_width(e, q.scene, 0), q.scene, pl.path.arg[2])) &&
                   (pl.extend.none() || engine_accepts(engine_of_width(e, q.scene, width), q.scene, pl.extend.arg[2])) &&
                   (pl.shadow_key.none() || engine_accepts(engine_of_width(e, q.scene, width), q.scene, shadow_cold));
-  if (!ok) { pl.path = pl.extend = pl.shade = pl.shade_early = pl.shadow_key = pl.volume_key = pl.shadow_volume_key = InstanceKey{}; pl.slim_state = false; pl.camera_trace = false; pl.camera_mode = 0; pl.camera_vertex = false; }
+  if (!ok) { pl.path = pl.extend = pl.shade = pl.shade_early = pl.shadow_key = pl.volume_key = pl.shadow_volume_key = InstanceKey{}; pl.slim_state = false; pl.camera_trace = false; pl.camera_mode = 0; pl.camera_vertex = false; pl.pixel_table = false; pl.cull_root_lds = false; }
   out = pl;
   return ok ? CRT_OK : CRT_ERR_UNSUPPORTED;
 }
@@ -490,6 +497,8 @@
   int slim_state = 1;
   int camera_trace = -1;
   int camera_vertex = -1;
+  int pixel_table = -1;
+  int cull_root_lds = -1;
   int noclassify_from = 1 << 30, tail_from = 12, lanes = 4, grid_mult = 0;
   size_t max_batch_slots = 0, lane_min_paths = (size_t)96 << 20, stage_min_paths = (size_t)96 << 20;
 };
diff --git a/crust-render_amd/csrc/kernels/camera_pixel.hip.h b/crust-render_amd/csrc/kernels/camera_pixel.hip.h
--- /dev/null
+++ b/crust-render_amd/csrc/kernels/camera_pixel.hip.h
@@ -0,0 +1,47 @@
+#pragma once
+
+#include "qmc.hip.h"
+
+namespace crt {
+namespace dev {
+
+constexpr int kDomainCamera = 0, kDomainPath = 1;
+
+struct PixelRec {
+  float px, py;
+  uint32_t seed[5];
+  uint32_t path_pattern;
+};
+static_assert(sizeof(PixelRec) == 32, "two 16-byte loads per camera sample");
+constexpr uint32_t kPixelTableMaxExtent = 1u << 24;
+
+__device__ __forceinline__ Sampler pixel_root(uint32_t px, uint32_t py, int frame, int index) {
+  const int tile = (int)(px >> 8) + (int)(py >> 8) * 4096;
+  return new_domain(sampler_new((int)px, (int)py, frame, index), tile);
+}
+__device__ __forceinline__ PixelRec pixel_record(uint32_t lin, uint32_t width, int frame) {
+  const uint32_t px = lin % width, py = lin / width;
+  const Sampler root = pixel_root(px, py, frame, 0);
+  PixelRec r;
+  r.px = (float)px; r.py = (float)py;
+  owen_seeds(new_domain(root, kDomainCamera).pattern, r.seed);
+  r.path_pattern = new_domain(root, kDomainPath).pattern;
+  return r;
+}
+
+struct SampleCursor { uint32_t pix, sl, step_pix, step_sl; };
+__device__ __forceinline__ SampleCursor sample_cursor(unsigned long long g, unsigned long long step, uint32_t n_act) {
+  SampleCursor c;
+  c.pix = (uint32_t)(g % n_act); c.sl = (uint32_t)(g / n_act);
+  c.step_pix = (uint32_t)(step % n_act); c.step_sl = (uint32_t)(step / n_act);
+  return c;
+}
+__device__ __forceinline__ void sample_cursor_next(SampleCursor &c, uint32_t n_act) {
+  const uint32_t room = n_act - c.step_pix;
+  const bool wrap = c.pix >= room;
+  c.pix = wrap ? c.pix - room : c.pix + c.step_pix;
+  c.sl += c.step_sl + (wrap ? 1u : 0u);
+}
+
+}
+}
diff --git a/crust-render_amd/csrc/kernels/pathtrace.hip b/crust-render_amd/csrc/kernels/pathtrace.hip
--- a/crust-render_amd/csrc/kernels/pathtrace.hip
+++ b/crust-render_amd/csrc/kernels/pathtrace.hip
@@ -6,6 +6,7 @@
 #include <unordered_map>
 #include <vector>
 
+#include "camera_pixel.hip.h"
 #include "shade.hip.h"
 #include "traverse_camera.hip.h"
 #include "traverse_pool.hip.h"
@@ -29,6 +30,7 @@
 #endif
 
 enum { K_CAMERA = 0, K_PATH = 1, K_TIME = 2 };
+static_assert(K_CAMERA == kDomainCamera && K_PATH == kDomainPath, "camera_pixel.hip.h derives the same domains");
 constexpr uint32_t kFilmTarget = 0x80000000u;
 constexpr uint32_t kPrevValid = 1u << 16, kPrevDelta = 1u << 17;
 constexpr int kMediumShift = 18;
@@ -317,6 +319,45 @@
   return ((k / kBlock) * (size_t)gridDim.x + blockIdx.x) * kBlock + (k % kBlock);
 }
 
+__device__ __forceinline__ void pixel_rec_load(const Params &P, const PixelRec *table, uint32_t pix, uint4 &r0, uint4 &r1) {
+  const uint4 *rec = reinterpret_cast<const uint4 *>(table + (P.active ? P.active[pix] : pix));
+  r0 = rec[0]; r1 = rec[1];
+}
+__device__ __forceinline__ CameraSample camera_sample_table(const Params &P, uint4 r0, uint4 r1, uint32_t pix, uint32_t sl,
+                                                            uint32_t sample_begin, const uint32_t *sobol_tab) {
+  CameraSample cs;
+  cs.pix = pix; cs.sl = sl;
+  const uint32_t seed[5] = {r0.z, r0.w, r1.x, r1.y, r1.z};
+  float cam[4];
+  draw_sample4_seeded(sample_begin + sl, seed, cam, sobol_tab);
+  const float fx = filter_offset(P.filter_kind, P.filter_radius, cam[0]);
+  const float fy = filter_offset(P.filter_kind, P.filter_radius, cam[1]);
+  const float u = (__uint_as_float(r0.x) + fx) / (float)P.width;
+  const float v = (__uint_as_float(r0.y) + fy) / (float)P.height;
+  cs.time = 0.0f;
+  camera_get_ray(P.camera, u, v, cam[2], cam[3], cs.o, cs.d);
+  cs.pattern = r1.w;
+  return cs;
+}
+__device__ __forceinline__ bool root_touched_lds(const uint32_t *node, V3 o, V3 d) {
+  const float4 *nb = reinterpret_cast<const float4 *>(node);
+  float bmin[3][4], bmax[3][4];
+#pragma unroll
+  for (int a = 0; a < 3; a++) {
+    const float4 lo = nb[a], hi = nb[3 + a];
+    bmin[a][0] = lo.x; bmin[a][1] = lo.y; bmin[a][2] = lo.z; bmin[a][3] = lo.w;
+    bmax[a][0] = hi.x; bmax[a][1] = hi.y; bmax[a][2] = hi.z; bmax[a][3] = hi.w;
+  }
+  const uint4 ch = *reinterpret_cast<const uint4 *>(nb + 6);
+  const uint32_t child[4] = {ch.x, ch.y, ch.z, ch.w};
+  return node_touched(bmin, bmax, child, o.x, o.y, o.z, d.x, d.y, d.z, 0.001f, CRT_INF);
+}
+__global__ void k_fill_pixel_table(const uint32_t *pixel_index, uint32_t n_pix, uint32_t width, int frame, PixelRec *table) {
+  const uint32_t i = blockIdx.x * blockDim.x + threadIdx.x;
+  if (i >= n_pix) return;
+  table[i] = pixel_record(pixel_index[i], width, frame);
+}
+
 template <bool PLANE_D>
 __device__ __forceinline__ void compact_camera_path(const Params &P, uint32_t k, float4 a, float4 &A, float4 &B, uint4 &D) {
   const V3 o = ld3(P.camera.origin) + splat(0.0f);
@@ -448,15 +489,17 @@
 
 constexpr int kCamLdsDwords = kCamWindow * kLdsNodeStride + kCamStack * kBlock;
 static_assert((kSobolLdsWords + kCamLdsDwords) * 4 + 512 <= 40 * 1024, "four workgroups of k_camera per CU");
+template <bool TABLE, bool ROOT_LDS>
 __global__ __launch_bounds__(kBlock, 4) void k_camera(Params P, PathSoA S, uint32_t *defer_plane, HitSoA H, Counters *C,
-                                                      uint32_t sample_begin, uint32_t n_samples, float4 *staging, uint32_t mode) {
+                                                      uint32_t sample_begin, uint32_t n_samples, float4 *staging, uint32_t mode,
+                                                      const PixelRec *pixel_table) {
   __shared__ uint32_t sobol_tab[kSobolLdsWords];
   __shared__ __attribute__((aligned(16))) uint32_t cam_lds[kCamLdsDwords];
   __shared__ uint32_t cam_ctr[3];
   const bool cull = P.root_cull != 0;
-  float bmin[3][4], bmax[3][4];
-  uint32_t child[4];
-  {
+  float bmin[3][4] = {}, bmax[3][4] = {};
+  uint32_t child[4] = {};
+  if (!ROOT_LDS) {
     const WideNode &root = P.scene.nodes[P.scene.root];
 #pragma unroll
     for (int a = 0; a < 3; a++)
@@ -479,18 +522,32 @@
   uint32_t *list = defer_plane + 4 * seg0;
   const V3 cam_o = ld3(P.camera.origin) + splat(0.0f);
   uint32_t n_culled = 0, n_valid = 0;
+  SampleCursor at_g = {0, 0, 0, 0};
+  uint4 rec0 = make_uint4(0, 0, 0, 0), rec1 = make_uint4(0, 0, 0, 0);
+  if (TABLE) {
+    at_g = sample_cursor(camera_slot_sample(threadIdx.x), (unsigned long long)gridDim.x * kBlock, P.n_act);
+    pixel_rec_load(P, pixel_table, at_g.pix, rec0, rec1);
+  }
   for (size_t k0 = 0; k0 < P.seg_cap; k0 += kBlock) {
     if (camera_slot_sample(k0) >= total) break;
     const size_t g = camera_slot_sample(k0 + threadIdx.x);
+    const uint32_t t_pix = at_g.pix, t_sl = at_g.sl;
+    const uint4 t_rec0 = rec0, t_rec1 = rec1;
+    if (TABLE) {
+      sample_cursor_next(at_g, P.n_act);
+      pixel_rec_load(P, pixel_table, at_g.pix, rec0, rec1);
+    }
     CameraSample cs;
     cs.o = splat(0.0f); cs.d = splat(0.0f); cs.time = 0.0f; cs.pattern = 0; cs.pix = 0; cs.sl = 0;
     bool keep = false;
     if (g < total) {
-      cs = camera_sample(P, g, sample_begin, sobol_tab);
+      if (TABLE) cs = camera_sample_table(P, t_rec0, t_rec1, t_pix, t_sl, sample_begin, sobol_tab);
+      else cs = camera_sample(P, g, sample_begin, sobol_tab);
       keep = true;
       n_valid = (uint32_t)(k0 + threadIdx.x) + 1;
       if (cull) {
-        keep = node_touched(bmin, bmax, child, cs.o.x, cs.o.y, cs.o.z, cs.d.x, cs.d.y, cs.d.z, 0.001f, CRT_INF);
+        keep = ROOT_LDS ? root_touched_lds(lds_nodes + (size_t)P.scene.root * kLdsNodeStride, cs.o, cs.d)
+                        : node_touched(bmin, bmax, child, cs.o.x, cs.o.y, cs.o.z, cs.d.x, cs.d.y, cs.d.z, 0.001f, CRT_INF);
         if (!keep) {
           const V3 L = escaped_to_sky(cs.d, splat(1.0f), splat(0.0f));
           st_nt(&staging[cs.sl * P.n_act + cs.pix], make_float4(L.x, L.y, L.z, 0.0f));
@@ -1457,17 +1514,18 @@
 }
 
 static_assert((kSobolLdsWords + kCamLdsDwords + kPipeMatMax * kMatDwords) * 4 + 512 <= 40 * 1024, "four workgroups of k_camera_vertex per CU");
-template <bool DRV>
+template <bool DRV, bool TABLE, bool ROOT_LDS>
 __global__ __launch_bounds__(kBlock, 4) void k_camera_vertex(Params P, PathSoA S, PathSoA N, Counters *C, uint32_t sample_begin,
-                                                             uint32_t n_samples, float4 *staging, uint32_t mode, int slim_out) {
+                                                             uint32_t n_samples, float4 *staging, uint32_t mode, int slim_out,
+                                                             const PixelRec *pixel_table) {
   __shared__ uint32_t sobol_tab[kSobolLdsWords];
   __shared__ __attribute__((aligned(16))) uint32_t cam_lds[kCamLdsDwords];
   __shared__ __attribute__((aligned(16))) uint32_t mat_lds[kPipeMatMax * kMatDwords];
   __shared__ uint32_t cam_ctr[4];
   const bool cull = P.root_cull != 0;
-  float bmin[3][4], bmax[3][4];
-  uint32_t child[4];
-  {
+  float bmin[3][4] = {}, bmax[3][4] = {};
+  uint32_t child[4] = {};
+  if (!ROOT_LDS) {
     const WideNode &root = P.scene.nodes[P.scene.root];
 #pragma unroll
     for (int a = 0; a < 3; a++)
@@ -1495,9 +1553,21 @@
   const size_t seg0 = (size_t)blockIdx.x * kBins * P.seg_cap;
   const V3 cam_o = ld3(P.camera.origin) + splat(0.0f);
   uint32_t n_escaped = 0, n_vertices = 0;
+  SampleCursor at_g = {0, 0, 0, 0};
+  uint4 rec0 = make_uint4(0, 0, 0, 0), rec1 = make_uint4(0, 0, 0, 0);
+  if (TABLE) {
+    at_g = sample_cursor(camera_slot_sample(threadIdx.x), (unsigned long long)gridDim.x * kBlock, P.n_act);
+    pixel_rec_load(P, pixel_table, at_g.pix, rec0, rec1);
+  }
   for (size_t k0 = 0; k0 < P.seg_cap; k0 += kBlock) {
     if (camera_slot_sample(k0) >= total) break;
     const size_t g = camera_slot_sample(k0 + threadIdx.x);
+    const uint32_t t_pix = at_g.pix, t_sl = at_g.sl;
+    const uint4 t_rec0 = rec0, t_rec1 = rec1;
+    if (TABLE) {
+      sample_cursor_next(at_g, P.n_act);
+      pixel_rec_load(P, pixel_table, at_g.pix, rec0, rec1);
+    }
     CameraSample cs;
     cs.o = splat(0.0f); cs.d = splat(0.0f); cs.time = 0.0f; cs.pattern = 0; cs.pix = 0; cs.sl = 0;
     int res = CAM_MISS;
@@ -1505,10 +1575,13 @@
     VertexOut v;
     v.origin = splat(0.0f); v.dir = splat(0.0f); v.beta = splat(1.0f); v.L = splat(0.0f); v.delta = false;
     if (g < total) {
-      cs = camera_sample(P, g, sample_begin, sobol_tab);
+      if (TABLE) cs = camera_sample_table(P, t_rec0, t_rec1, t_pix, t_sl, sample_begin, sobol_tab);
+      else cs = camera_sample(P, g, sample_begin, sobol_tab);
       valid = true;
       bool keep = true;
-      if (cull) keep = node_touched(bmin, bmax, child, cs.o.x, cs.o.y, cs.o.z, cs.d.x, cs.d.y, cs.d.z, 0.001f, CRT_INF);
+      if (cull)
+        keep = ROOT_LDS ? root_touched_lds(lds_nodes + (size_t)P.scene.root * kLdsNodeStride, cs.o, cs.d)
+                        : node_touched(bmin, bmax, child, cs.o.x, cs.o.y, cs.o.z, cs.d.x, cs.d.y, cs.d.z, 0.001f, CRT_INF);
       float t = 0.0f;
       uint32_t prim = kInvalid;
       if (keep)
@@ -1743,7 +1816,10 @@
 using PathFn = void (*)(Params, PathSoA, PathSoA, HitSoA, ShadowSoA, Counters *, float4 *, uint32_t, uint32_t, uint32_t, int);
 using ShadeFn = void (*)(Params, PathSoA, PathSoA, HitSoA, ShadowSoA, Counters *, int, float4 *, int);
 using ShadePipeFn = void (*)(Params, PathSoA, PathSoA, HitSoA, Counters *, int, float4 *, int, uint32_t, int);
-using CameraVertexFn = void (*)(Params, PathSoA, PathSoA, Counters *, uint32_t, uint32_t, float4 *, uint32_t, int);
+using CameraVertexFn = void (*)(Params, PathSoA, PathSoA, Counters *, uint32_t, uint32_t, float4 *, uint32_t, int, const PixelRec *);
+using CameraFn = void (*)(Params, PathSoA, uint32_t *, HitSoA, Counters *, uint32_t, uint32_t, float4 *, uint32_t, const PixelRec *);
+template <bool TABLE, bool ROOT_LDS>
+static CameraVertexFn camera_vertex_fn(bool drv) { return drv ? k_camera_vertex<true, TABLE, ROOT_LDS> : k_camera_vertex<false, TABLE, ROOT_LDS>; }
 using ShadowFn = void (*)(Params, PathSoA, ShadowSoA, Counters *, float4 *, CrtTravStats *);
 using ShadeVolFn = void (*)(Params, PathSoA, PathSoA, HitSoA, ShadowSoA, Counters *, int, float4 *, int, uint32_t *);
 template <class Fn>
@@ -1829,6 +1905,7 @@
   CrtLight *d_lights = nullptr;
   std::vector<std::shared_ptr<void>> environments;
   uint32_t *d_pixels = nullptr;
+  PixelRec *d_pixel_table = nullptr;
   int grid = 768;
   hipStream_t last_stream = nullptr;
   bool profile = false;
@@ -1860,6 +1937,7 @@
     if (d_count) (void)hipFree(d_count);
     if (d_lights) (void)hipFree(d_lights);
     if (d_pixels) (void)hipFree(d_pixels);
+    if (d_pixel_table) (void)hipFree(d_pixel_table);
   }
 
   void drain_events() {
@@ -1988,16 +2066,42 @@
     return CRT_HIP_OK(hipGetLastError()) ? CRT_OK : fail(CRT_ERR_NO_DEVICE);
   }
 
-  int plan_lane(Lane &B, Params &p, uint32_t n_samples, bool stats) {
-    const size_t total = (size_t)p.n_act * n_samples;
-    in.total = total;
-    in.stats = stats;
+  void plan_inputs_from_params() {
     in.scene = P.scene;
     in.n_lights = P.n_lights; in.has_inf_lights = P.has_inf_lights != 0; in.has_env = P.envs != nullptr; in.strategy = P.strategy;
     in.has_motion = P.has_motion != 0; in.lens = P.camera.lens_radius > 0.0f;
     in.mat_index = P.mat_index != nullptr; in.partition = P.partition; in.n_materials = P.n_materials; in.max_depth = P.max_depth;
     in.class_stats = P.class_stats;
     in.volumes = volumes != nullptr;
+  }
+  void build_pixel_table() {
+    in.pixel_table_ready = false;
+    if (in.pixel_table_knob == 0 || P.width > kPixelTableMaxExtent || P.height > kPixelTableMaxExtent) return;
+    plan_inputs_from_params();
+    PlanInputs q = in;
+    q.total = ~(size_t)0 >> 1; q.stats = false; q.partial_active = false; q.pixel_table_ready = true;
+    LaunchPlan trial;
+    if (plan_launches(q, trial) != CRT_OK || !trial.pixel_table) return;
+    if (hipMalloc(&d_pixel_table, (size_t)P.n_pix * sizeof(PixelRec)) != hipSuccess) {
+      (void)hipGetLastError();
+      d_pixel_table = nullptr;
+      return;
+    }
+    hipLaunchKernelGGL(k_fill_pixel_table, dim3((P.n_pix + 255) / 256), dim3(256), 0, nullptr, P.pixel_index, P.n_pix, P.width,
+                       P.frame, d_pixel_table);
+    if (hipGetLastError() != hipSuccess || hipStreamSynchronize(nullptr) != hipSuccess) {
+      (void)hipFree(d_pixel_table);
+      d_pixel_table = nullptr;
+      return;
+    }
+    in.pixel_table_ready = true;
+  }
+
+  int plan_lane(Lane &B, Params &p, uint32_t n_samples, bool stats) {
+    const size_t total = (size_t)p.n_act * n_samples;
+    in.total = total;
+    in.stats = stats;
+    plan_inputs_from_params();
     in.partial_active = p.active != nullptr;
     if (in.volumes && stats) {
       set_error_text("render refused: the stats build does not run volume renders");
@@ -2072,16 +2176,22 @@
       timed(0, st, [&] { hipLaunchKernelGGL(path, dim3(grid), dim3(kBlock), 0, st, p, S[0], S[1], H, Q, C, staging, sample_begin, n_samples, 0u, 0); });
       return fold();
     }
+    const PixelRec *pixel_table = plan.pixel_table ? d_pixel_table : nullptr;
+    if (plan.pixel_table && !pixel_table) return CRT_ERR_UNSUPPORTED;
     Params p0 = p;
     if (plan.camera_vertex) {
       p0.cam_compact = 2;
       const uint32_t nx = 1;
       const int slim_out = (shade_slim && nx <= P.max_depth && nx < plan.tail_at && (int)nx < plan.noclassify_from) ? 1 : 0;
-      const CameraVertexFn fn = plan.shade_early.arg[0] ? k_camera_vertex<true> : k_camera_vertex<false>;
-      timed(3, st, [&] { hipLaunchKernelGGL(fn, dim3(grid), dim3(kBlock), 0, st, p, S[0], S[1], C, sample_begin, n_samples, staging, plan.camera_mode, slim_out); });
-    } else if (plan.camera_trace)
-      timed(3, st, [&] { hipLaunchKernelGGL(k_camera, dim3(grid), dim3(kBlock), 0, st, p, S[0], reinterpret_cast<uint32_t *>(S[1].a), H, C, sample_begin, n_samples, staging, plan.camera_mode); });
-    else
+      const bool drv = plan.shade_early.arg[0] != 0;
+      const CameraVertexFn fn = plan.pixel_table ? (plan.cull_root_lds ? camera_vertex_fn<true, true>(drv) : camera_vertex_fn<true, false>(drv))
+                                                 : (plan.cull_root_lds ? camera_vertex_fn<false, true>(drv) : camera_vertex_fn<false, false>(drv));
+      timed(3, st, [&] { hipLaunchKernelGGL(fn, dim3(grid), dim3(kBlock), 0, st, p, S[0], S[1], C, sample_begin, n_samples, staging, plan.camera_mode, slim_out, pixel_table); });
+    } else if (plan.camera_trace) {
+      const CameraFn fn = plan.pixel_table ? (plan.cull_root_lds ? k_camera<true, true> : k_camera<true, false>)
+                                           : (plan.cull_root_lds ? k_camera<false, true> : k_camera<false, false>);
+      timed(3, st, [&] { hipLaunchKernelGGL(fn, dim3(grid), dim3(kBlock), 0, st, p, S[0], reinterpret_cast<uint32_t *>(S[1].a), H, C, sample_begin, n_samples, staging, plan.camera_mode, pixel_table); });
+    } else
       timed(3, st, [&] { hipLaunchKernelGGL(k_generate, dim3(grid), dim3(kBlock), 0, st, p, S[0], C, sample_begin, n_samples, staging); });
     int cur = 0;
     for (uint32_t it = 0; it <= P.max_depth; it++) {
@@ -2322,6 +2432,9 @@
   in.shade_wide = knobs.shade_wide;
   in.force_fused = knobs.fused;
   in.stage_min_paths = knobs.stage_min_paths;
+  in.pixel_table_knob = knobs.pixel_table;
+  in.cull_root_lds_knob = knobs.cull_root_lds;
+  r.build_pixel_table();
   r.max_batch_slots = knobs.max_batch_slots;
   r.n_lanes = knobs.lanes < 1 ? 1 : (knobs.lanes > Renderer::kMaxLanes ? Renderer::kMaxLanes : knobs.lanes);
   r.lane_min_paths = knobs.lane_min_paths;
@@ -2490,7 +2603,8 @@
   const LaunchPlan &plan = r->r.last_plan;
   out[0] = plan.fused ? 1u : 0u;
   out[1] = (plan.wide ? 1u : 0u) | (plan.shade_piped() ? 2u : 0u) | (plan.root_cull ? 4u : 0u) | (plan.slim_state ? 8u : 0u) |
-           (plan.volumes ? 16u : 0u) | (plan.camera_trace ? 32u : 0u) | (plan.camera_vertex ? 64u : 0u);
+           (plan.volumes ? 16u : 0u) | (plan.camera_trace ? 32u : 0u) | (plan.camera_vertex ? 64u : 0u) |
+           (plan.pixel_table ? 128u : 0u) | (plan.cull_root_lds ? 256u : 0u);
   out[2] = (uint32_t)r->r.grid;
   return CRT_OK;
 }
diff --git a/crust-render_amd/csrc/kernels/qmc.hip.h b/crust-render_amd/csrc/kernels/qmc.hip.h
--- a/crust-render_amd/csrc/kernels/qmc.hip.h
+++ b/crust-render_amd/csrc/kernels/qmc.hip.h
@@ -80,6 +80,27 @@
     out[d] = unit_f32(x);
   }
 }
+__device__ __forceinline__ void owen_seeds(uint32_t pattern, uint32_t seed[5]) {
+  seed[0] = pcg_hash(pattern);
+#pragma unroll
+  for (int d = 0; d < 4; d++) seed[d + 1] = pcg_hash(pattern + (uint32_t)d + 1u);
+}
+__device__ __forceinline__ void draw_sample4_seeded(uint32_t index, const uint32_t seed[5], float out[4], const uint32_t *tab) {
+  const uint32_t idx = owen(index, seed[0]);
+  const uint32_t b0 = idx & 255u, b1 = (idx >> 8) & 255u, b2 = (idx >> 16) & 255u, b3 = idx >> 24;
+#pragma unroll
+  for (int d = 0; d < 4; d++) {
+    uint32_t x;
+    if (d == 0) {
+      x = __brev(idx);
+    } else {
+      const uint32_t *t = tab + (d - 1) * 1024;
+      x = t[b0] ^ t[256 + b1] ^ t[512 + b2] ^ t[768 + b3];
+    }
+    x = owen(x, seed[d + 1]);
+    out[d] = unit_f32(x);
+  }
+}
 __device__ __forceinline__ float draw_rnd1(Sampler s) {
   return unit_f32(pcg_hash(s.pattern ^ (s.index * 0x9e3779b9u + 0x7f4a7c15u)));
 }
diff --git a/crust-render_amd/csrc/scene.cpp b/crust-render_amd/csrc/scene.cpp
--- a/crust-render_amd/csrc/scene.cpp
+++ b/crust-render_amd/csrc/scene.cpp
@@ -224,6 +224,8 @@
   if (num("CRT_SLIM_STATE", v)) k.slim_state = v != 0;
   if (num("CRT_CAMERA_TRACE", v)) k.camera_trace = (v >= 0 && v <= 3) ? (int)v : 1;
   if (num("CRT_CAMERA_VERTEX", v)) k.camera_vertex = v != 0 ? 1 : 0;
+  if (num("CRT_PIXEL_TABLE", v)) k.pixel_table = v != 0 ? 1 : 0;
+  if (num("CRT_CULL_ROOT_LDS", v)) k.cull_root_lds = v != 0 ? 1 : 0;
   if (num("CRT_FUSED", v)) k.fused = v != 0;
   if (num("CRT_NOCLASSIFY_FROM", v)) k.noclassify_from = (int)std::min<long long>(std::max<long long>(v, 0), 1 << 30);
   if (num("CRT_TAIL_FROM", v)) k.tail_from = (int)std::min<long long>(std::max<long long>(v, 0), 1 << 30);
```

Result: faster. 12740 Mray/s, median of 6 (+2.5%).
